# FaspDevTeam/faspsolver

Hardware: AMD Instinct MI355X
Metric: AMG-PCG solve DOF/s (3D 7-pt Poisson 256^3, classical AMG V(1,1) w-Jacobi + PCG, rtol 1e-8) (higher is better)
Workload: dtype f64

## Files before the change

### faspsolver_amd/__init__.py

```python
import ctypes as C
import os
import subprocess

import numpy as np

from . import _types as T
from ._types import *

_HERE = os.path.dirname(os.path.abspath(__file__))
LIB_PATH = os.environ.get("FASP_HIP_LIB") or os.path.join(_HERE, "libfasp_hip.so")
_lib = None

EXPORTS = [
    "fasp_param_amg_init", "fasp_param_solver_init", "fasp_solver_dcsr_krylov_amg",
    "fasp_blas_dcsr_mxv", "fasp_blas_dcsr_aAxpy", "fasp_blas_darray_dotprod",
    "fasp_blas_darray_norm2", "fasp_blas_darray_norminf", "fasp_blas_darray_axpy",
    "fasp_blas_darray_axpby", "fasp_smoother_dcsr_jacobi",
    "fasp_blas_dbsr_mxv", "fasp_blas_dbsr_aAxpy", "fasp_dbsr_getdiaginv", "fasp_smoother_dbsr_jacobi1",
    "fasp_solver_dbsr_pcg", "fasp_solver_dbsr_pbcgs", "fasp_solver_dbsr_pgmres", "fasp_solver_dbsr_pvgmres",
    "fasp_solver_dbsr_pvfgmres", "fasp_hip_bsr_precond_setup", "fasp_hip_bsr_precond_fct", "fasp_hip_bsr_precond_free",
    "fasp_hip_param_input", "fasp_fwrapper_dcsr_krylov_amg_", "fasp_dcsrvec_read2", "fasp_dvec_read",
    "fasp_dbsr_read", "fasp_dcoo_read", "fasp_dcoo_read1", "fasp_dcoo_shift_read", "fasp_dmtx_read", "fasp_dmtxsym_read", "fasp_dvec_write", "fasp_dcsr_write_coo", "fasp_dcsrvec_write2", "fasp_fwrapper_dcsr_amg_", "fasp_fwrapper_dbsr_krylov_amg_", "fasp_hip_free_bsr", "fasp_hip_comm_selftest", "fasp_hip_amg_kernel_info", "fasp_hip_coarse_kernel_info", "fasp_hip_bsr_coarse_kernel_info", "fasp_hip_coding_selftest", "fasp_solver_amg", "fasp_solver_famg", "fasp_hip_amg_solve", "fasp_precond_diag", "fasp_precond_dbsr_diag", "fasp_solver_dcsr_itsolver", "fasp_solver_dcsr_krylov", "fasp_solver_dcsr_krylov_diag", "fasp_solver_dbsr_itsolver", "fasp_solver_dbsr_krylov", "fasp_solver_dbsr_krylov_diag", "fasp_hip_mxv_csr", "fasp_hip_mxv_bsr", "fasp_solver_matfree_init", "fasp_solver_pcg", "fasp_solver_pbcgs", "fasp_solver_pgcg", "fasp_solver_pminres", "fasp_solver_pgmres", "fasp_solver_pvgmres", "fasp_solver_pvfgmres", "fasp_solver_itsolver", "fasp_solver_krylov", "fasp_solver_dcsr_pcg", "fasp_solver_dcsr_pminres", "fasp_solver_dcsr_pgcg", "fasp_solver_dcsr_pgcr", "fasp_solver_dcsr_pbcgs", "fasp_solver_dcsr_pgmres", "fasp_solver_dcsr_pvgmres",
    "fasp_solver_dcsr_pvfgmres", "fasp_hip_precond_setup", "fasp_hip_precond_fct", "fasp_hip_precond_free",
    "fasp_hip_time_bsr_mxv", "fasp_solver_dbsr_krylov_amg", "fasp_hip_bsr_amg_create", "fasp_hip_bsr_amg_create_host",
    "fasp_hip_bsr_amg_destroy", "fasp_hip_bsr_amg_num_levels", "fasp_hip_bsr_amg_get_matrix",
    "fasp_hip_bsr_amg_get_diaginv", "fasp_hip_bsr_solve",
    "fasp_hip_set_device", "fasp_hip_device_count", "fasp_hip_device_identity", "fasp_hip_available",
    "fasp_hip_amg_create", "fasp_hip_amg_create_host", "fasp_hip_amg_upload",
    "fasp_hip_amg_destroy", "fasp_hip_amg_num_levels", "fasp_hip_amg_get_matrix",
    "fasp_hip_amg_get_cfmark", "fasp_hip_solve", "fasp_hip_set_rhs", "fasp_hip_set_guess",
    "fasp_hip_solve_resident", "fasp_hip_get_solution", "fasp_hip_device_synchronize",
    "fasp_hip_precond_amg",
    "fasp_hip_poisson7pt", "fasp_hip_aniso27pt", "fasp_hip_free_system", "fasp_hip_time_kernel", "fasp_hip_measure_ceilings", "fasp_hip_amg_publish", "fasp_hip_amg_attach", "fasp_hip_amg_unpublish",
    "fasp_precond_setup", "fasp_precond_amg", "fasp_precond_famg", "fasp_precond_amli", "fasp_precond_namli", "fasp_amg_data_create", "fasp_amg_data_free", "fasp_param_amg_to_prec", "fasp_param_prec_to_amg", "fasp_mem_free", "fasp_mem_calloc", "fasp_dvec_alloc", "fasp_dvec_set", "fasp_dvec_free", "fasp_dvec_create", "fasp_dcsr_create", "fasp_dcsr_free", "fasp_smoother_dcsr_gs", "fasp_smoother_dcsr_sor", "fasp_smoother_dcsr_L1diag",
    "fasp_hip_tune", "fasp_hip_comm_unique_id", "fasp_hip_comm_init", "fasp_hip_comm_finalize",
    "fasp_hip_comm_rank", "fasp_hip_comm_size", "fasp_hip_version", "fasp_hip_comm_init_shm",
    "fasp_hip_dist_plan", "fasp_hip_dist_level_info", "fasp_hip_dist_get_matrix",
    "fasp_hip_dist_get_list",
    "fasp_blas_dcsr_vmv", "fasp_blas_dcsr_mxv_agg", "fasp_blas_dcsr_aAxpy_agg", "fasp_blas_darray_ax",
    "fasp_blas_darray_axpyz", "fasp_blas_darray_norm1", "fasp_darray_cp", "fasp_darray_set", "fasp_dvec_isnan",
    "fasp_hip_time_matrix", "fasp_hip_bsr_dist_info", "fasp_hip_seq_schedule_selftest", "fasp_hip_seq_chain_selftest", "fasp_hip_cluster_order", "fasp_hip_permute_csr", "fasp_hip_comm_init_ipc", "fasp_hip_comm_stats", "fasp_hip_comm_timing", "fasp_hip_estream_selftest", "fasp_hip_sell_selftest", "fasp_hip_csr_plan", "fasp_hip_level_op", "fasp_hip_matrix_op", "fasp_hip_matrix_traits",
    "fasp_param_ilu_init", "fasp_ilu_data_create", "fasp_ilu_data_free", "fasp_mem_iludata_check", "fasp_ilu_dcsr_setup",
    "fasp_precond_ilu", "fasp_precond_ilu_forward", "fasp_precond_ilu_backward", "fasp_solver_dcsr_krylov_ilu",
    "fasp_solver_dcsr_krylov_ilu_M", "fasp_smoother_dcsr_ilu", "fasp_fwrapper_dcsr_krylov_ilu_",
    "fasp_hip_ilu_resident_count", "fasp_hip_ilu_time",
    "fasp_ilu_dbsr_setup", "fasp_precond_dbsr_ilu", "fasp_solver_dbsr_krylov_ilu", "fasp_smoother_dbsr_ilu",
    "fasp_fwrapper_dbsr_krylov_ilu_",
    "fasp_hip_bsr_amg_get_ilu", "fasp_hip_bsr_amg_ilu_info", "fasp_hip_bsr_amg_ilu_smooth_time",
    "fasp_hip_bsr_sweep", "fasp_hip_csr_sweep",
    "fasp_blas_dcsr_rap", "fasp_hip_dcsr_rap", "fasp_hip_rap_info", "fasp_hip_rap_device_count", "fasp_hip_rap_time",
    "fasp_dstr_create", "fasp_dstr_alloc", "fasp_dstr_free", "fasp_dstr_cp", "fasp_format_dstr_dcsr", "fasp_dstr_read",
    "fasp_blas_dstr_aAxpy", "fasp_blas_dstr_mxv", "fasp_precond_dstr_diag", "fasp_solver_dstr_pcg", "fasp_solver_dstr_pbcgs",
    "fasp_solver_dstr_pminres", "fasp_solver_dstr_pgmres", "fasp_solver_dstr_pvgmres", "fasp_solver_dstr_itsolver",
    "fasp_solver_dstr_krylov", "fasp_solver_dstr_krylov_diag", "fasp_hip_mxv_str", "fasp_hip_str_form", "fasp_hip_time_str_mxv",
    "fasp_ilu_dstr_setup0", "fasp_ilu_dstr_setup1", "fasp_precond_dstr_ilu0", "fasp_precond_dstr_ilu1", "fasp_solver_dstr_krylov_ilu",
    "fasp_hip_str_ilu_form", "fasp_hip_str_ilu_apply", "fasp_hip_time_str_ilu",
    "fasp_smoother_dstr_jacobi", "fasp_smoother_dstr_jacobi1", "fasp_smoother_dstr_gs", "fasp_smoother_dstr_gs1",
    "fasp_smoother_dstr_gs_ascend", "fasp_smoother_dstr_gs_descend", "fasp_smoother_dstr_gs_order", "fasp_smoother_dstr_gs_cf",
    "fasp_smoother_dstr_sor", "fasp_smoother_dstr_sor1", "fasp_smoother_dstr_sor_ascend", "fasp_smoother_dstr_sor_descend",
    "fasp_smoother_dstr_sor_order", "fasp_smoother_dstr_sor_cf",
    "fasp_hip_str_sweep", "fasp_hip_str_sweep_form", "fasp_hip_str_sweep_levels", "fasp_hip_time_str_sweep",
    "fasp_generate_diaginv_block", "fasp_smoother_dstr_swz", "fasp_precond_dstr_blockgs", "fasp_solver_dstr_krylov_blockgs",
    "fasp_hip_str_swz", "fasp_hip_str_swz_levels", "fasp_hip_time_str_swz",
    "fasp_param_swz_init", "fasp_dcsr_sympart", "fasp_dcsr_shift", "fasp_sparse_mis", "fasp_swz_dcsr_setup", "fasp_dcsr_swz_forward",
    "fasp_dcsr_swz_backward", "fasp_precond_swz", "fasp_swz_data_free", "fasp_solver_dcsr_krylov_swz",
    "fasp_hip_csr_swz_levels", "fasp_hip_csr_swz", "fasp_hip_csr_swz_resident_count", "fasp_hip_time_csr_swz",
    "fasp_hip_csr_swz_runs", "fasp_hip_amg_get_swz", "fasp_hip_amg_swz_info", "fasp_hip_amg_swz_sweep_time", "fasp_hip_amg_swz_levels",
]


def build(verbose=False):
    cmd = ["make", "-C", os.path.join(_HERE, "csrc")]
    if not verbose:
        cmd.insert(1, "-s")
    subprocess.run(cmd, check=True)


def lib():
    global _lib
    if _lib is not None:
        return _lib
    if not os.path.exists(LIB_PATH):
        build()
    L = C.CDLL(LIB_PATH)
    P = C.POINTER
    L.fasp_param_amg_init.argtypes = [P(T.AMG_param)]
    L.fasp_param_solver_init.argtypes = [P(T.ITS_param)]
    L.fasp_solver_dcsr_krylov_amg.argtypes = [P(T.dCSRmat), P(T.dvector), P(T.dvector),
                                              P(T.ITS_param), P(T.AMG_param)]
    L.fasp_blas_dcsr_mxv.argtypes = [P(T.dCSRmat), T.c_double_p, T.c_double_p]
    L.fasp_blas_dcsr_aAxpy.argtypes = [C.c_double, P(T.dCSRmat), T.c_double_p, T.c_double_p]
    for f in ("fasp_blas_darray_dotprod", "fasp_blas_darray_norm2", "fasp_blas_darray_norminf"):
        getattr(L, f).restype = C.c_double
    L.fasp_blas_darray_dotprod.argtypes = [C.c_int, T.c_double_p, T.c_double_p]
    L.fasp_blas_darray_norm2.argtypes = [C.c_int, T.c_double_p]
    L.fasp_blas_darray_norminf.argtypes = [C.c_int, T.c_double_p]
    L.fasp_blas_darray_axpy.argtypes = [C.c_int, C.c_double, T.c_double_p, T.c_double_p]
    L.fasp_blas_darray_axpby.argtypes = [C.c_int, C.c_double, T.c_double_p, C.c_double,
                                         T.c_double_p]
    L.fasp_blas_dcsr_vmv.restype = C.c_double
    L.fasp_blas_dcsr_vmv.argtypes = [P(T.dCSRmat), T.c_double_p, T.c_double_p]
    L.fasp_blas_dcsr_mxv_agg.argtypes = [P(T.dCSRmat), T.c_double_p, T.c_double_p]
    L.fasp_blas_dcsr_aAxpy_agg.argtypes = [C.c_double, P(T.dCSRmat), T.c_double_p, T.c_double_p]
    L.fasp_blas_darray_ax.argtypes = [C.c_int, C.c_double, T.c_double_p]
    L.fasp_blas_darray_axpyz.argtypes = [C.c_int, C.c_double, T.c_double_p, T.c_double_p, T.c_double_p]
    L.fasp_blas_darray_norm1.restype = C.c_double
    L.fasp_blas_darray_norm1.argtypes = [C.c_int, T.c_double_p]
    L.fasp_darray_cp.argtypes = [C.c_int, T.c_double_p, T.c_double_p]
    L.fasp_darray_set.argtypes = [C.c_int, T.c_double_p, C.c_double]
    L.fasp_hip_time_matrix.restype = C.c_double
    L.fasp_hip_time_matrix.argtypes = [P(T.dCSRmat), C.c_int, C.c_int, P(C.c_int)]
    L.fasp_dvec_isnan.restype = C.c_short
    L.fasp_dvec_isnan.argtypes = [P(T.dvector)]
    L.fasp_smoother_dcsr_jacobi.argtypes = [P(T.dvector), C.c_int, C.c_int, C.c_int,
                                            P(T.dCSRmat), P(T.dvector), C.c_int, C.c_double]
    L.fasp_blas_dbsr_mxv.argtypes = [P(T.dBSRmat), T.c_double_p, T.c_double_p]
    L.fasp_blas_dbsr_aAxpy.argtypes = [C.c_double, P(T.dBSRmat), T.c_double_p, T.c_double_p]
    L.fasp_dbsr_getdiaginv.argtypes = [P(T.dBSRmat)]
    L.fasp_dbsr_getdiaginv.restype = T.dvector
    L.fasp_smoother_dbsr_jacobi1.argtypes = [P(T.dBSRmat), P(T.dvector), P(T.dvector), T.c_double_p]
    L.fasp_hip_bsr_sweep.argtypes = [P(T.dBSRmat), T.c_double_p, T.c_double_p, T.c_double_p, C.c_int, C.c_int, C.c_double,
                                     P(C.c_int)]
    L.fasp_hip_csr_sweep.argtypes = [P(T.dCSRmat), P(C.c_int), C.c_int, C.c_int, C.c_double, C.c_int, T.c_double_p, T.c_double_p,
                                     P(C.c_int)]
    L.fasp_hip_time_bsr_mxv.argtypes = [P(T.dBSRmat), C.c_int]
    L.fasp_hip_time_bsr_mxv.restype = C.c_double
    L.fasp_solver_dcsr_pcg.argtypes = [P(T.dCSRmat), P(T.dvector), P(T.dvector), P(T.precond), C.c_double,
                                       C.c_double, C.c_int, C.c_short, C.c_short]
    L.fasp_solver_dcsr_pbcgs.argtypes = L.fasp_solver_dcsr_pcg.argtypes
    L.fasp_solver_dcsr_pminres.argtypes = L.fasp_solver_dcsr_pcg.argtypes
    L.fasp_solver_dcsr_pgcg.argtypes = L.fasp_solver_dcsr_pcg.argtypes
    L.fasp_solver_dcsr_pvgmres.argtypes = [P(T.dCSRmat), P(T.dvector), P(T.dvector), P(T.precond), C.c_double,
                                           C.c_double, C.c_int, C.c_short, C.c_short, C.c_short]
    L.fasp_solver_dcsr_pvfgmres.argtypes = L.fasp_solver_dcsr_pvgmres.argtypes
    L.fasp_solver_dcsr_pgmres.argtypes = L.fasp_solver_dcsr_pvgmres.argtypes
    L.fasp_solver_dcsr_pgcr.argtypes = L.fasp_solver_dcsr_pvgmres.argtypes
    L.fasp_hip_precond_setup.argtypes = [P(T.dCSRmat), P(T.AMG_param)]
    L.fasp_hip_precond_setup.restype = P(T.precond)
    L.fasp_hip_precond_free.argtypes = [P(T.precond)]
    L.fasp_hip_precond_free.restype = None
    L.fasp_hip_precond_fct.argtypes = [T.c_double_p, T.c_double_p, C.c_void_p]
    L.fasp_hip_precond_fct.restype = None
    L.fasp_solver_dbsr_pcg.argtypes = [P(T.dBSRmat), P(T.dvector), P(T.dvector), P(T.precond), C.c_double,
                                       C.c_double, C.c_int, C.c_short, C.c_short]
    L.fasp_solver_dbsr_pbcgs.argtypes = L.fasp_solver_dbsr_pcg.argtypes
    L.fasp_solver_dbsr_pvgmres.argtypes = [P(T.dBSRmat), P(T.dvector), P(T.dvector), P(T.precond), C.c_double,
                                           C.c_double, C.c_int, C.c_short, C.c_short, C.c_short]
    L.fasp_solver_dbsr_pgmres.argtypes = L.fasp_solver_dbsr_pvgmres.argtypes
    L.fasp_solver_dbsr_pvfgmres.argtypes = L.fasp_solver_dbsr_pvgmres.argtypes
    L.fasp_hip_bsr_precond_setup.argtypes = [P(T.dBSRmat), P(T.AMG_param)]
    L.fasp_hip_bsr_precond_setup.restype = P(T.precond)
    L.fasp_hip_bsr_precond_free.argtypes = [P(T.precond)]
    L.fasp_hip_bsr_precond_free.restype = None
    L.fasp_hip_bsr_precond_fct.argtypes = [T.c_double_p, T.c_double_p, C.c_void_p]
    L.fasp_hip_bsr_precond_fct.restype = None
    L.fasp_dcsrvec_read2.argtypes = [C.c_char_p, C.c_char_p, P(T.dCSRmat), P(T.dvector)]
    L.fasp_dvec_read.argtypes = [C.c_char_p, P(T.dvector)]
    L.fasp_dbsr_read.argtypes = [C.c_char_p, P(T.dBSRmat)]
    L.fasp_hip_free_bsr.argtypes = [P(T.dBSRmat)]
    L.fasp_hip_free_bsr.restype = None
    L.fasp_hip_param_input.argtypes = [C.c_char_p, P(T.ITS_param), P(T.AMG_param)]
    L.fasp_fwrapper_dcsr_krylov_amg_.argtypes = [P(C.c_int), P(C.c_int), T.c_int_p, T.c_int_p, T.c_double_p,
                                                 T.c_double_p, T.c_double_p, P(C.c_double), P(C.c_int), P(C.c_int)]
    L.fasp_fwrapper_dcsr_krylov_amg_.restype = None
    L.fasp_hip_coding_selftest.argtypes = [P(T.dCSRmat), P(C.c_int)]
    L.fasp_hip_amg_kernel_info.argtypes = [C.c_void_p, C.c_int, C.c_int, P(C.c_int), P(C.c_double)]
    L.fasp_hip_coarse_kernel_info.argtypes = [C.c_void_p, P(C.c_int)]
    L.fasp_hip_bsr_coarse_kernel_info.argtypes = [C.c_void_p, P(C.c_int)]
    L.fasp_solver_amg.argtypes = [P(T.dCSRmat), P(T.dvector), P(T.dvector), P(T.AMG_param)]
    L.fasp_hip_amg_solve.argtypes = [C.c_void_p, P(T.dvector), P(T.dvector), P(T.AMG_param), T.c_double_p,
                                     C.c_int, P(T.fasp_hip_stats)]
    L.fasp_solver_dbsr_krylov_amg.argtypes = [P(T.dBSRmat), P(T.dvector), P(T.dvector), P(T.ITS_param),
                                              P(T.AMG_param)]
    L.fasp_hip_bsr_amg_create.argtypes = [P(C.c_void_p), P(T.dBSRmat), P(T.AMG_param)]
    L.fasp_hip_bsr_amg_create_host.argtypes = [P(C.c_void_p), P(T.dBSRmat), P(T.AMG_param)]
    L.fasp_hip_bsr_amg_destroy.argtypes = [C.c_void_p]
    L.fasp_hip_bsr_amg_destroy.restype = None
    L.fasp_hip_bsr_amg_num_levels.argtypes = [C.c_void_p]
    L.fasp_hip_bsr_amg_get_matrix.argtypes = [C.c_void_p, C.c_int, C.c_int, P(T.dBSRmat)]
    L.fasp_hip_bsr_amg_get_diaginv.argtypes = [C.c_void_p, C.c_int]
    L.fasp_hip_bsr_amg_get_diaginv.restype = T.c_double_p
    L.fasp_hip_bsr_solve.argtypes = [C.c_void_p, P(T.dvector), P(T.dvector), P(T.ITS_param), T.c_double_p,
                                     C.c_int, P(T.fasp_hip_stats)]
    L.fasp_hip_amg_create.argtypes = [P(C.c_void_p), P(T.dCSRmat), P(T.AMG_param)]
    L.fasp_hip_amg_create_host.argtypes = L.fasp_hip_amg_create.argtypes
    L.fasp_hip_amg_upload.argtypes = [C.c_void_p]
    L.fasp_hip_amg_destroy.argtypes = [C.c_void_p]
    L.fasp_hip_amg_destroy.restype = None
    L.fasp_hip_amg_num_levels.argtypes = [C.c_void_p]
    L.fasp_hip_amg_get_matrix.argtypes = [C.c_void_p, C.c_int, C.c_int, P(T.dCSRmat)]
    L.fasp_hip_amg_get_cfmark.argtypes = [C.c_void_p, C.c_int, P(T.ivector)]
    L.fasp_hip_solve.argtypes = [C.c_void_p, P(T.dvector), P(T.dvector), P(T.ITS_param),
                                 T.c_double_p, C.c_int, P(T.fasp_hip_stats)]
    L.fasp_hip_set_rhs.argtypes = [C.c_void_p, P(T.dvector)]
# ... 606 lines not shown
```

### faspsolver_amd/csrc/device_csr.hip.h

```cpp

struct DevCSR {
    int     row = 0, col = 0, nnz = 0;
    int*    ia  = nullptr;
    int*    ja  = nullptr;
    double* val = nullptr;
    int*    dpos = nullptr;
    bool    dup_diag = false;
    bool    sorted = false;
    int     lanes = 8;
    int     kind = 0;
    int     tile_rows = 256;
    int     wrows = 64, wcap = 512;
    unsigned char* code = nullptr;
    int*    rowbase = nullptr;
    int*    doff = nullptr;
    double* dval = nullptr;
    unsigned short* pat = nullptr;
    int*    pstart = nullptr;
    int*    plen = nullptr;
    int*    poff = nullptr;
    double* pval = nullptr;
    int     npat = 0, npent = 0;
    unsigned short* ja16 = nullptr;
    int*            jbase = nullptr;
    int     nxrows = -1;
    int     plane = 0;
    int     win_lo = 0, win_hi = -1;
    unsigned short* lja16 = nullptr;
    int*    tptr = nullptr;
    int*    tcols = nullptr;
    long long ntcols = 0;
    const int* bridge = nullptr;
    double*    bscratch = nullptr;
    int        bridge_dir = 0;
    int*       es_tab = nullptr;
    unsigned short* es_ja16 = nullptr;
    double*    es_part = nullptr;
    int        es_W = 0, es_nc = 0;
    unsigned*      sell_code = nullptr;
    int*           sell_meta = nullptr;
    unsigned char* sell_rlen = nullptr;
    double*        sell_tab = nullptr;
    int            sell_nv = 0, sell_obits = 0, sell_nslice = 0;
    long long      sell_slots = 0;
    void    release()
    {
        if (sell_code) (void)hipFree(sell_code);
        if (sell_meta) (void)hipFree(sell_meta);
        if (sell_rlen) (void)hipFree(sell_rlen);
        if (sell_tab) (void)hipFree(sell_tab);
        sell_code = nullptr; sell_meta = nullptr; sell_rlen = nullptr; sell_tab = nullptr; sell_nv = sell_obits = sell_nslice = 0; sell_slots = 0;
        if (es_tab) (void)hipFree(es_tab);
        if (es_part) (void)hipFree(es_part);
        if (es_ja16) (void)hipFree(es_ja16);
        es_tab = nullptr; es_part = nullptr; es_ja16 = nullptr; es_W = es_nc = 0;
        if (bscratch) (void)hipFree(bscratch);
        bscratch = nullptr; bridge = nullptr; bridge_dir = 0;
        if (lja16) (void)hipFree(lja16);
        if (tptr) (void)hipFree(tptr);
        if (tcols) (void)hipFree(tcols);
        lja16 = nullptr; tptr = nullptr; tcols = nullptr;
        nxrows = -1;
        if (ja16) (void)hipFree(ja16);
        ja16 = nullptr;
        if (jbase) (void)hipFree(jbase);
        jbase = nullptr;
        if (ia) (void)hipFree(ia);
        if (ja) (void)hipFree(ja);
        if (val) (void)hipFree(val);
        if (dpos) (void)hipFree(dpos);
        if (code) (void)hipFree(code);
        if (rowbase) (void)hipFree(rowbase);
        if (doff) (void)hipFree(doff);
        if (dval) (void)hipFree(dval);
        if (pat) (void)hipFree(pat);
        if (pstart) (void)hipFree(pstart);
        if (plen) (void)hipFree(plen);
        if (poff) (void)hipFree(poff);
        if (pval) (void)hipFree(pval);
        pat = nullptr; pstart = plen = poff = nullptr; pval = nullptr;
        ia = ja = dpos = rowbase = doff = nullptr; val = dval = nullptr; code = nullptr;
    }
};

static void pick_kernel(DevCSR& M)
{
    const double avg = M.row > 0 ? (double)M.nnz / M.row : 1.0;
    static const double stream_max = std::getenv("FASP_HIP_STREAM_MAX") ? std::atof(std::getenv("FASP_HIP_STREAM_MAX")) : 48.0;
    M.kind = avg <= stream_max ? 2 : 0;
    M.lanes = avg < 300.0 ? 16 : avg < 1000.0 ? 32 : 64;
    while (M.lanes < 64 && (double)M.row * M.lanes < 0.75 * MAXGRID * BLOCK) M.lanes *= 2;
    if (avg < 48.0) M.lanes = avg < 3.0 ? 2 : avg < 6.0 ? 4 : avg < 24.0 ? 8 : 16;
    static const int small_rows = std::getenv("FASP_HIP_SMALL_XFER_ROWS") ? std::atoi(std::getenv("FASP_HIP_SMALL_XFER_ROWS")) : 256 * 1024;
    if (M.kind == 2 && M.row != M.col && M.row < small_rows) M.kind = 0;
    int R = 256;
    while (R < STREAM_MAXR && R * 2 * avg <= 3072.0) R <<= 1;
    M.tile_rows = R;
    M.wrows = 64;
    M.wcap  = 512;
}

static bool g_oneshot_upload = false;
static bool compress_enabled()
{
    if (g_oneshot_upload) return false;
    static int en = -1;
    if (en < 0) { const char* e = std::getenv("FASP_HIP_COMPRESS"); en = (e && std::atoi(e) == 0) ? 0 : 1; }
    return en != 0;
}
struct PairKey { int off; unsigned long long bits; };
static inline unsigned pair_hash(int off, unsigned long long bits)
{
    unsigned long long h = bits * 0x9E3779B97F4A7C15ull + (unsigned long long)(unsigned)off * 0xC2B2AE3D27D4EB4Full;
    return (unsigned)(h >> 40);
}
static bool build_dict8(const HostCSR& M, std::vector<int>& doff, std::vector<double>& dval,
                        Buf<unsigned char>& code, Buf<int>& rowbase)
{
    const bool square = M.row == M.col;
    const int n = M.row;
    if (n <= 0 || M.nnz <= 0) return false;
    constexpr int SLOTS = 1024;
    struct Table {
        int      cnt = 0;
        int      slot_id[SLOTS];
        PairKey  keys[257];
        Table() { for (int& s : slot_id) s = -1; }
        int find_or_add(int off, unsigned long long bits, bool add)
        {
            unsigned h = pair_hash(off, bits) & (SLOTS - 1);
            for (;;) {
                const int id = slot_id[h];
                if (id < 0) {
                    if (!add || cnt >= 257) return -1;
                    keys[cnt] = PairKey{off, bits};
                    slot_id[h] = cnt;
                    return cnt++;
                }
                if (keys[id].off == off && keys[id].bits == bits) return id;
                h = (h + 1) & (SLOTS - 1);
            }
        }
    };
    auto base_of = [&](int r) { return square ? r : (M.ia[r] < M.ia[r + 1] ? M.ja[M.ia[r]] : 0); };
    auto bits_of = [](double v) { unsigned long long b; std::memcpy(&b, &v, 8); return b; };
    const int nt = omp_get_max_threads();
    std::vector<Table> local((size_t)nt);
    bool fail = false;
#pragma omp parallel num_threads(nt)
    {
        Table& T = local[(size_t)omp_get_thread_num()];
#pragma omp for schedule(static)
        for (int r = 0; r < n; ++r) {
            if (fail || T.cnt > 256) continue;
            const int base = base_of(r);
            for (int k = M.ia[r]; k < M.ia[r + 1]; ++k)
                if (T.find_or_add(M.ja[k] - base, bits_of(M.val[k]), true) < 0 || T.cnt > 256) { fail = true; break; }
        }
    }
    if (fail) return false;
    std::vector<PairKey> all;
    for (const Table& T : local) all.insert(all.end(), T.keys, T.keys + T.cnt);
    std::sort(all.begin(), all.end(), [](const PairKey& x, const PairKey& y) {
        return x.off != y.off ? x.off < y.off : x.bits < y.bits; });
    all.erase(std::unique(all.begin(), all.end(), [](const PairKey& x, const PairKey& y) {
        return x.off == y.off && x.bits == y.bits; }), all.end());
    if (all.size() > 256) return false;
    doff.assign(256, 0); dval.assign(256, 0.0);
    Table G;
    for (size_t i = 0; i < all.size(); ++i) {
        G.find_or_add(all[i].off, all[i].bits, true);
        doff[i] = all[i].off;
        std::memcpy(&dval[i], &all[i].bits, 8);
    }
    code.alloc((size_t)M.nnz);
    if (!square) rowbase.alloc((size_t)n);
#pragma omp parallel
    {
        Table T = G;
#pragma omp for schedule(static)
        for (int r = 0; r < n; ++r) {
            const int base = base_of(r);
            if (!square) rowbase[r] = base;
            for (int k = M.ia[r]; k < M.ia[r + 1]; ++k)
                code[k] = (unsigned char)T.find_or_add(M.ja[k] - base, bits_of(M.val[k]), false);
        }
    }
    return true;
}

static bool build_rowpat(const HostCSR& M, Buf<unsigned short>& pat, std::vector<int>& pstart, std::vector<int>& plen,
                         std::vector<int>& poff, std::vector<double>& pval, Buf<int>& rowbase)
{
    const bool square = M.row == M.col || M.row_aligned;
    const int n = M.row;
    if (n <= 0 || M.nnz <= 0) return false;
    if ((long long)M.col >= (1ll << 28)) return false;
    constexpr int MAXPAT = 65535, MAXENT = 1 << 20;
    auto base_of = [&](int r) { return square ? r : (M.ia[r] < M.ia[r + 1] ? M.ja[M.ia[r]] : 0); };
// ... 478 lines not shown
    const int ns = (n + 63) / 64;
    S.rlen.assign((size_t)n, 0);
    S.sptr.assign((size_t)ns + 1, 0);
    int toolong = 0;
#pragma omp parallel for schedule(static) reduction(+ : toolong)
    for (int s = 0; s < ns; ++s) {
        int W = 0;
        for (int r = s * 64; r < std::min(n, s * 64 + 64); ++r) {
            const int len = M.ia[r + 1] - M.ia[r];
            if (len > 255) { ++toolong; continue; }
            S.rlen[(size_t)r] = (unsigned char)len;
            W = std::max(W, len);
        }
        S.sptr[(size_t)s + 1] = W;
    }
    if (toolong) { why = 2; return false; }
    long long wsum = 0;
    for (int s = 0; s < ns; ++s) wsum += S.sptr[(size_t)s + 1];
    S.nslice = ns;
    S.slots = 64ll * wsum;
    if (S.slots * 100 > (long long)cap_percent * M.nnz || wsum >= (1ll << 30)) { why = 3; return false; }
    for (int s = 0; s < ns; ++s) S.sptr[(size_t)s + 1] += S.sptr[(size_t)s];
    constexpr int VSLOTS = 32768;
    struct VSet {
        std::vector<unsigned long long> key;
        std::vector<long long> cnt;
        std::vector<int> id;
        int n = 0;
        VSet() : key((size_t)VSLOTS, 0ull), cnt((size_t)VSLOTS, 0), id((size_t)VSLOTS, -1) {}
        static unsigned slot_of(unsigned long long b) { return (unsigned)((b * 0x9E3779B97F4A7C15ull) >> 49); }
        bool add(unsigned long long b, long long c)
        {
            unsigned s = slot_of(b);
            for (;;) {
                if (cnt[s] == 0) {
                    if (n >= SELL_MAXV) return false;
                    key[s] = b; cnt[s] = c; ++n;
                    return true;
                }
                if (key[s] == b) { cnt[s] += c; return true; }
                s = (s + 1) & (VSLOTS - 1);
            }
        }
        int slot(unsigned long long b) const
        {
            unsigned s = slot_of(b);
            for (;;) {
                if (cnt[s] == 0) return -1;
                if (key[s] == b) return (int)s;
                s = (s + 1) & (VSLOTS - 1);
            }
        }
    };
    auto bits_of = [](double v) { unsigned long long b; std::memcpy(&b, &v, 8); return b; };
    const int nt = std::max(1, std::min(omp_get_max_threads(), n / 4096 + 1));
    std::vector<VSet*> local((size_t)nt, nullptr);
    bool fail = false;
#pragma omp parallel num_threads(nt)
    {
        VSet* T = new VSet();
        local[(size_t)omp_get_thread_num()] = T;
#pragma omp for schedule(static)
        for (int r = 0; r < n; ++r) {
            if (fail) continue;
            for (int k = M.ia[r]; k < M.ia[r + 1]; ++k)
                if (!T->add(bits_of(M.val[k]), 1)) { fail = true; break; }
        }
    }
    VSet Gs;
    for (VSet* T : local) {
        if (T && !fail)
            for (int s = 0; s < VSLOTS && !fail; ++s)
                if (T->cnt[(size_t)s] && !Gs.add(T->key[(size_t)s], T->cnt[(size_t)s])) fail = true;
        delete T;
    }
    if (fail) { why = 4; return false; }
    std::vector<std::pair<long long, unsigned long long>> order;
    for (int s = 0; s < VSLOTS; ++s)
        if (Gs.cnt[(size_t)s]) order.emplace_back(-Gs.cnt[(size_t)s], Gs.key[(size_t)s]);
    std::sort(order.begin(), order.end());
    S.nv = (int)order.size();
    S.tab.resize(order.size());
    for (size_t i = 0; i < order.size(); ++i) std::memcpy(&S.tab[i], &order[i].second, 8);
    for (size_t i = 0; i < order.size(); ++i) Gs.id[(size_t)Gs.slot(order[i].second)] = (int)i;
    S.vbits = 0;
    while ((1ll << S.vbits) < S.nv) ++S.vbits;
    S.sbase.assign((size_t)ns, 0);
    int maxoff = 0;
#pragma omp parallel for schedule(static) reduction(max : maxoff)
    for (int s = 0; s < ns; ++s) {
        const int k0 = M.ia[s * 64], k1 = M.ia[std::min(n, s * 64 + 64)];
        if (k1 <= k0) continue;
        int lo = M.ja[k0], hi = lo;
        for (int k = k0 + 1; k < k1; ++k) { lo = std::min(lo, M.ja[k]); hi = std::max(hi, M.ja[k]); }
        S.sbase[(size_t)s] = lo;
        maxoff = std::max(maxoff, hi - lo);
    }
    S.obits = 1;
    while ((1ll << S.obits) <= maxoff) ++S.obits;
    if (S.vbits + S.obits > 32) { why = 5; return false; }
    S.code.alloc((size_t)std::max<long long>(S.slots, 1));
    bool lost = false;
#pragma omp parallel for schedule(static)
    for (int s = 0; s < ns; ++s) {
        const int W = S.sptr[(size_t)s + 1] - S.sptr[(size_t)s], base = S.sbase[(size_t)s];
        unsigned* cs = S.code.data() + (size_t)S.sptr[(size_t)s] * 64;
        for (int l = 0; l < 64; ++l) {
            const int r = s * 64 + l;
            const int kb = r < n ? M.ia[r] : 0, len = r < n ? M.ia[r + 1] - kb : 0;
            for (int k = 0; k < len; ++k) {
                const int sl = Gs.slot(bits_of(M.val[kb + k]));
                if (sl < 0) { lost = true; continue; }
                const int id = Gs.id[(size_t)sl];
                cs[(size_t)k * 64 + l] = ((unsigned)id << S.obits) | (unsigned)(M.ja[kb + k] - base);
            }
            for (int k = len; k < W; ++k) cs[(size_t)k * 64 + l] = 0u;
        }
    }
    if (lost) { why = 4; return false; }
    why = 0;
    return true;
}

static void sell_mxv_host(const SellHost& S, int nrow, const double* x, double* y)
{
    const unsigned omask = (1u << S.obits) - 1u;
    for (int s = 0; s < S.nslice; ++s) {
        const int W = S.sptr[(size_t)s + 1] - S.sptr[(size_t)s], base = S.sbase[(size_t)s];
        const unsigned* cs = S.code.data() + (size_t)S.sptr[(size_t)s] * 64;
        double acc[64];
        for (int l = 0; l < 64; ++l) acc[l] = 0.0;
        for (int k = 0; k < W; ++k)
            for (int l = 0; l < 64; ++l) {
                const int r = s * 64 + l;
                if (r >= nrow || k >= (int)S.rlen[(size_t)r]) continue;
                const unsigned c = cs[(size_t)k * 64 + l];
                acc[l] = acc[l] + S.tab[c >> S.obits] * x[base + (int)(c & omask)];
            }
        for (int l = 0; l < 64 && s * 64 + l < nrow; ++l) y[s * 64 + l] = acc[l];
    }
}
static void sell_decode_host(const SellHost& S, int nrow, int* ia, int* ja, double* val)
{
    const unsigned omask = (1u << S.obits) - 1u;
    ia[0] = 0;
    for (int r = 0; r < nrow; ++r) ia[r + 1] = ia[r] + (int)S.rlen[(size_t)r];
    for (int r = 0; r < nrow; ++r) {
        const int s = r >> 6, l = r & 63, base = S.sbase[(size_t)s];
        const unsigned* cs = S.code.data() + (size_t)S.sptr[(size_t)s] * 64;
        for (int k = 0; k < (int)S.rlen[(size_t)r]; ++k) {
            const unsigned c = cs[(size_t)k * 64 + l];
            ja[ia[r] + k] = base + (int)(c & omask);
            val[ia[r] + k] = S.tab[c >> S.obits];
        }
    }
}

static int upload_sell(const HostCSR& H, DevCSR& D)
{
    static const bool on = !(std::getenv("FASP_HIP_SELL") && std::atoi(std::getenv("FASP_HIP_SELL")) == 0);
    if (!on) return FASP_SUCCESS;
    static const bool timing = std::getenv("FASP_HIP_SETUP_TIMING") != nullptr;
    const double t0 = wall_seconds();
    SellHost S;
    int why = 0;
    const bool ok = build_sell(H, S, SELL_CAP_PERCENT, &why);
    if (timing) std::printf("        [sell %d x %d, %d nnz] %s (%d) %d values, %d + %d bits, %.3f slots per entry, %.3f s\n", H.row, H.col, H.nnz,
                            ok ? "coded" : "not coded", why, S.nv, S.vbits, S.obits, (double)S.slots / std::max(H.nnz, 1), wall_seconds() - t0);
    if (!ok) return FASP_SUCCESS;
    const size_t ns = (size_t)S.nslice;
    std::vector<int> meta(2 * ns + 1);
    std::copy(S.sptr.begin(), S.sptr.end(), meta.begin());
    std::copy(S.sbase.begin(), S.sbase.end(), meta.begin() + (long)ns + 1);
    HIPCK(hipMalloc(&D.sell_code, sizeof(unsigned) * (size_t)std::max<long long>(S.slots, 1)));
    HIPCK(hipMalloc(&D.sell_meta, sizeof(int) * meta.size()));
    HIPCK(hipMalloc(&D.sell_rlen, (size_t)H.row));
    HIPCK(hipMalloc(&D.sell_tab, sizeof(double) * (size_t)S.nv));
    HIPCK(hipMemcpy(D.sell_code, S.code.data(), sizeof(unsigned) * (size_t)S.slots, hipMemcpyHostToDevice));
    HIPCK(hipMemcpy(D.sell_meta, meta.data(), sizeof(int) * meta.size(), hipMemcpyHostToDevice));
    HIPCK(hipMemcpy(D.sell_rlen, S.rlen.data(), (size_t)H.row, hipMemcpyHostToDevice));
    HIPCK(hipMemcpy(D.sell_tab, S.tab.data(), sizeof(double) * (size_t)S.nv, hipMemcpyHostToDevice));
    D.sell_nv = S.nv; D.sell_obits = S.obits; D.sell_nslice = S.nslice; D.sell_slots = S.slots;
    return FASP_SUCCESS;
}

static int upload_csr(const HostCSR& H, DevCSR& D)
{
    D.row = H.row; D.col = H.col; D.nnz = H.nnz;
    HIPCK(hipMalloc(&D.ia, sizeof(int) * ((size_t)H.row + 1)));
    HIPCK(hipMalloc(&D.ja, sizeof(int) * std::max<size_t>(H.nnz, 1)));
    HIPCK(hipMalloc(&D.val, sizeof(double) * (std::max<size_t>(H.nnz, 1) + 2)));
    HIPCK(hipMemsetAsync(D.val + std::max<size_t>(H.nnz, 1), 0, sizeof(double) * 2, g_ctx.stream));
    HIPCK(hipMemcpyAsync(D.ia, H.ia.data(), sizeof(int) * ((size_t)H.row + 1), hipMemcpyHostToDevice, g_ctx.stream));
    pick_kernel(D);
    auto upload_plain = [&]() -> int {
        HIPCK(hipMemcpyAsync(D.ja, H.ja.data(), sizeof(int) * (size_t)H.nnz, hipMemcpyHostToDevice, g_ctx.stream));
        HIPCK(hipMemcpyAsync(D.val, H.val.data(), sizeof(double) * (size_t)H.nnz, hipMemcpyHostToDevice, g_ctx.stream));
        return 0;
    };
    if (compress_enabled() && H.nnz >= 4096 && (double)H.nnz <= 48.0 * H.row) {
        Buf<unsigned short> pat; Buf<int> prb;
        std::vector<int> pstart, plen, poff; std::vector<double> pval;
        static const bool rowpat_on = !(std::getenv("FASP_HIP_ROWPAT") && std::atoi(std::getenv("FASP_HIP_ROWPAT")) == 0);
        if (rowpat_on && build_rowpat(H, pat, pstart, plen, poff, pval, prb)) {
            D.npat = (int)pstart.size(); D.npent = (int)poff.size();
            HIPCK(hipMalloc(&D.pat, sizeof(unsigned short) * ((size_t)H.row + 2)));
            HIPCK(hipMalloc(&D.pstart, sizeof(int) * pstart.size()));
            HIPCK(hipMalloc(&D.plen, sizeof(int) * plen.size()));
            HIPCK(hipMemcpy(D.plen, plen.data(), sizeof(int) * plen.size(), hipMemcpyHostToDevice));
            HIPCK(hipMalloc(&D.poff, sizeof(int) * std::max<size_t>(poff.size(), 1)));
            HIPCK(hipMalloc(&D.pval, sizeof(double) * std::max<size_t>(pval.size(), 1)));
            HIPCK(hipMemset(D.pat + H.row, 0xff, sizeof(unsigned short) * 2));
            HIPCK(hipMemcpy(D.pat, pat.data(), sizeof(unsigned short) * (size_t)H.row, hipMemcpyHostToDevice));
            HIPCK(hipMemcpy(D.pstart, pstart.data(), sizeof(int) * pstart.size(), hipMemcpyHostToDevice));
            HIPCK(hipMemcpy(D.poff, poff.data(), sizeof(int) * poff.size(), hipMemcpyHostToDevice));
            HIPCK(hipMemcpy(D.pval, pval.data(), sizeof(double) * pval.size(), hipMemcpyHostToDevice));
            if (prb.n) {
                HIPCK(hipMalloc(&D.rowbase, sizeof(int) * ((size_t)H.row + 2)));
                HIPCK(hipMemcpy(D.rowbase, prb.data(), sizeof(int) * (size_t)H.row, hipMemcpyHostToDevice));
                const int nr = H.row, npair = (nr + 1) / 2;
                long long nx = 0;
#pragma omp parallel for schedule(static) reduction(+ : nx)
                for (int w0 = 0; w0 < nr; w0 += 128) {
                    const int    pm = std::min((w0 + 64) / 2, npair - 1);
                    const unsigned domA = pat[(size_t)2 * pm], domB = (2 * pm + 1 < nr) ? pat[(size_t)2 * pm + 1] : 0xffffu;
                    for (int r = w0; r < std::min(w0 + 128, nr); r += 2) {
                        const bool vb = r + 1 < nr;
                        if (!(vb && pat[r] == domA && pat[r + 1] == domB)) nx += vb ? 2 : 1;
                    }
                }
                if (nx * 4 <= nr) D.nxrows = (int)nx;
            } else {
                D.plane = grid_plane_of(poff, H.row);
                if (std::getenv("FASP_HIP_SETUP_TIMING")) std::printf("        [upload_csr %d x %d, %d nnz] %d row patterns; grid plane for the XCD strips: %d rows\n", H.row, H.col, H.nnz, (int)pstart.size(), D.plane);
                const int nr = H.row, npair = (nr + 1) / 2;
                long long nx = 0;
#pragma omp parallel for schedule(static) reduction(+ : nx)
                for (int w0 = 0; w0 < nr; w0 += 128) {
                    const unsigned dom = pat[(size_t)2 * std::min((w0 + 64) / 2, npair - 1)];
                    for (int r = w0; r < std::min(w0 + 128, nr); r += 2) {
                        const bool vb = r + 1 < nr;
                        if (!(vb && pat[r] == dom && pat[r + 1] == dom)) nx += vb ? 2 : 1;
                    }
                }
                if (nx * 4 <= nr) D.nxrows = (int)nx;
            }
            D.kind = 2;
            return upload_plain() < 0 ? ERROR_ALLOC_MEM : FASP_SUCCESS;
        }
        std::vector<int> doff; std::vector<double> dval;
        Buf<unsigned char> code; Buf<int> rowbase;
        if (build_dict8(H, doff, dval, code, rowbase)) {
            HIPCK(hipMalloc(&D.code, (size_t)H.nnz + 256));
            HIPCK(hipMalloc(&D.doff, sizeof(int) * 256));
            HIPCK(hipMalloc(&D.dval, sizeof(double) * 256));
            HIPCK(hipMemcpy(D.code, code.data(), (size_t)H.nnz, hipMemcpyHostToDevice));
            HIPCK(hipMemcpy(D.doff, doff.data(), sizeof(int) * 256, hipMemcpyHostToDevice));
            HIPCK(hipMemcpy(D.dval, dval.data(), sizeof(double) * 256, hipMemcpyHostToDevice));
            if (rowbase.n) {
                HIPCK(hipMalloc(&D.rowbase, sizeof(int) * (size_t)H.row));
                HIPCK(hipMemcpy(D.rowbase, rowbase.data(), sizeof(int) * (size_t)H.row, hipMemcpyHostToDevice));
            }
            D.kind = 2;
            return upload_plain() < 0 ? ERROR_ALLOC_MEM : FASP_SUCCESS;
        }
    }
    static const bool sort_long = !(std::getenv("FASP_HIP_SORT_LONG_ROWS") && std::atoi(std::getenv("FASP_HIP_SORT_LONG_ROWS")) == 0);
    static const int  sort_stream = std::getenv("FASP_HIP_SORT_STREAM") ? std::atoi(std::getenv("FASP_HIP_SORT_STREAM")) : 0;
    const double avg_len = H.row > 0 ? (double)H.nnz / H.row : 0.0;
    const bool do_sort = sort_long && !g_oneshot_upload && H.nnz > 0 && (D.kind == 0 || (D.kind == 2 && sort_stream > 0 && avg_len >= sort_stream));
    static const bool timing = std::getenv("FASP_HIP_SETUP_TIMING") != nullptr;
    double tp = wall_seconds();
    auto lap = [&](const char* what) {
        if (!timing) return;
        const double now = wall_seconds();
        std::printf("        [upload_csr %d x %d, %d nnz] %-10s %8.3f s\n", H.row, H.col, H.nnz, what, now - tp);
        tp = now;
    };
    if (do_sort && D.kind == 0) {
        int maxlen = 0;
#pragma omp parallel for schedule(static) reduction(max : maxlen)
        for (int i = 0; i < H.row; ++i) maxlen = std::max(maxlen, H.ia[i + 1] - H.ia[i]);
        if (g_device_sort && maxlen <= SORT_MAXLEN) {
            const int st = upload_sorted_on_device(H, D, maxlen);
            lap("device sort");
            return st < 0 ? st : build_estream(H.ia.data(), H.row, H.nnz, D);
        }
    }
    if (do_sort) {
        Buf<int> sj((size_t)H.nnz);
        Buf<double> sv((size_t)H.nnz);
        std::vector<int> dp;
        const bool square = H.row == H.col;
        if (square) dp.assign((size_t)H.row, -1);
#pragma omp parallel
        {
            std::vector<std::pair<int, double>> tmp;
#pragma omp for schedule(dynamic, 64)
            for (int i = 0; i < H.row; ++i) {
                const int kb = H.ia[i], ke = H.ia[i + 1];
                tmp.resize((size_t)(ke - kb));
                for (int k = kb; k < ke; ++k) tmp[(size_t)(k - kb)] = {H.ja[k], H.val[k]};
                std::stable_sort(tmp.begin(), tmp.end(),
                                 [](const std::pair<int, double>& x, const std::pair<int, double>& y) { return x.first < y.first; });
                for (int k = kb; k < ke; ++k) {
                    sj[k] = tmp[(size_t)(k - kb)].first; sv[k] = tmp[(size_t)(k - kb)].second;
                    if (square && sj[k] == i) dp[(size_t)i] = k;
                }
            }
        }
        lap("row sort");
        HIPCK(hipMemcpy(D.ja, sj.data(), sizeof(int) * (size_t)H.nnz, hipMemcpyHostToDevice));
        HIPCK(hipMemcpy(D.val, sv.data(), sizeof(double) * (size_t)H.nnz, hipMemcpyHostToDevice));
        lap("memcpy");
        if (square && D.kind == 2) {
            HIPCK(hipMalloc(&D.dpos, sizeof(int) * (size_t)std::max(H.row, 1)));
            HIPCK(hipMemcpy(D.dpos, dp.data(), sizeof(int) * (size_t)H.row, hipMemcpyHostToDevice));
        }
        D.sorted = true;
        if (upload_ja16(D, H.ia.data(), sj.data()) < 0) return ERROR_ALLOC_MEM;
        return build_estream(H.ia.data(), H.row, H.nnz, D);
    }
    if (upload_plain() < 0) return ERROR_ALLOC_MEM;
    if (D.kind == 2 && !g_oneshot_upload && build_xtile(H, D) < 0) return ERROR_ALLOC_MEM;
    if (D.kind == 2 && compress_enabled() && upload_sell(H, D) < 0) return ERROR_ALLOC_MEM;
    if (upload_ja16(D, H.ia.data(), H.ja.data()) < 0) return ERROR_ALLOC_MEM;
    return build_estream(H.ia.data(), H.row, H.nnz, D);
}

struct Tuning { int swz_run = -1, swz_run_width = 16, ilu_smooth_fused = 1, gen2 = 2, ws2_bpc = 3, maxgrid = -1, xcd = 16, nt = 1, kind = -1, lanes = -1, wrows = -1, wcap = -1, compress = 1, rpl = -1, lds_tab = 1, xcd_pat = 64, spcg_batch = 16, small_lds = 1, ja16 = 1, spcg_fused = 1, spcg_grid = 0, spcg_persist = 1, split_rows = 0, gs_multicolor = 0, seq_flow = 1, seq_strip_kb = 0, seq_jobs = 1, seq_spine = 1, seq_grid = 0, seq_chain = 1, seq_chain_n1 = 0, seq_chain_grid = 0, seq_chain_ref = 0, seq_test_hang = 0, seq_rest_lanes = 0, local_square = 1, fuse_zr = 1, fuse_presmooth = 1, seq_lanes = 0, xtile = 1, rp5_max = 45, rp_bpc = 5, rp_xcd = -1, rp_strip = 2, spcg_test_hang = 0, small_onewave = 4, lazy_coarse = 1, rp_stream = -1, renumber = 1, renumber_chunk = 262144, pcg_dev_beta = 1, spcg_spec = 1, ev_every = 4, pcg_fold = 1, seq_chain_touch = 8, seq_chain_touch_t1 = 1, seq_zero_skip = 1, estream = 1, es_dbg = 0, ilu_form = -1, str_ilu_form = -1, str_ilu_wgs = 0, str_sweep_form = -1, str_sweep_wgs = 0, sell = 1; };
static Tuning g_tune;

template <class K>
static int resident_blocks_per_cu(K kernel)
{
    static std::vector<std::pair<const void*, int>> cache;
    const void* key = reinterpret_cast<const void*>(kernel);
    for (const auto& e : cache)
        if (e.first == key) return e.second;
    int nb = 0;
    if (hipOccupancyMaxActiveBlocksPerMultiprocessor(&nb, kernel, BLOCK, 0) != hipSuccess || nb < 1) nb = 4;
    nb = std::min(nb, 8);
    cache.emplace_back(key, nb);
    return nb;
}

template <class K>
static int launch_persistent(K kernel, int ntiles, CsrArgs& a, int blocks_per_cu = 0)
{
    int cap = (blocks_per_cu > 0 ? std::min(blocks_per_cu, resident_blocks_per_cu(kernel)) : resident_blocks_per_cu(kernel)) * g_ctx.num_cu;
    if (g_tune.maxgrid > 0) cap = g_tune.maxgrid;
    cap = std::min(cap, MAXGRID);
    int grid = std::min(cap, ntiles);
    grid = std::max(8, (grid + 7) / 8 * 8);
    hipLaunchKernelGGL(kernel, dim3(grid), dim3(BLOCK), 0, g_ctx.stream, a);
    return grid;
}

enum CsrKernel : int {
    CK_ROWS_2 = 0, CK_ROWS_4, CK_ROWS_8, CK_ROWS_16, CK_ROWS_32, CK_ROWS_64,
    CK_WSTREAM_64_512, CK_WSTREAM_64_1024, CK_WSTREAM_32_512, CK_WSTREAM_32_1024,
    CK_ROWPAT_0_1, CK_ROWPAT_0_2, CK_ROWPAT_1_1, CK_ROWPAT_1_2, CK_ROWPAT_2_1, CK_ROWPAT_2_2,
    CK_DICT8_8, CK_DICT8_16, CK_DICT8_24,
    CK_ESTREAM_4, CK_ESTREAM_8, CK_ESTREAM_16, CK_ESTREAM_32,
    CK_ROWPAT4, CK_ROWPAT5, CK_LSTREAM, CK_XTILE, CK_SELL, CK_WSTREAM2
};
struct CsrPlan {
    CsrKernel kernel;
    int    family;
    int    tile_rows;
    int    bpc;
    int    xcd_map;
    int    tpp;
    int    nt;
    bool   ja16, jbase;
    bool   fused_zr;
    double bytes;
};
static CsrPlan plan_csr(const DevCSR& M, int op, bool windowed, bool want_partials, int rows = -1)
{
    CsrPlan p{};
    int kind = M.kind;
    if (rows < 0) rows = M.row;
    if (M.code && g_tune.compress) kind = 4;
    if (M.pat && g_tune.compress) kind = 5;
    if (g_tune.kind >= 0 && !(g_tune.kind == 4 && !M.code) && !(g_tune.kind == 5 && !M.pat)) kind = g_tune.kind;
    const int lanes = g_tune.lanes > 0 ? g_tune.lanes : M.lanes, wrows = g_tune.wrows > 0 ? g_tune.wrows : M.wrows, wcap = g_tune.wcap > 0 ? g_tune.wcap : M.wcap;
    const bool jac = op == OP_JACOBI, w64 = wrows == 64 && wcap == 512;
    const bool lstream_ok = g_tune.gen2 && kind == 2 && w64 && (double)M.nnz <= 7.6 * M.row;
    if (jac && kind != 0 && kind < 4 && (M.dup_diag || !M.dpos) && !lstream_ok) kind = 0;
    p.xcd_map = g_tune.xcd;
    p.nt = g_tune.nt | ((g_tune.rp_stream > 0 || (g_tune.rp_stream < 0 && (size_t)M.row * 8 > (size_t)96 << 20)) ? 4 : 0);
    p.ja16 = g_tune.ja16 && M.ja16; p.jbase = g_tune.ja16 && M.jbase;
    if (M.jbase && kind != 0) p.ja16 = p.jbase = false;
    if (kind == 1 || kind == 3) kind = 0;
    p.tile_rows = kind >= 4 ? BLOCK : kind == 2 ? 4 * wrows : BLOCK / lanes;
    auto ntiles = [&] { return (rows + p.tile_rows - 1) / p.tile_rows; };
    auto strips = [&] {
        const int rpb = p.tile_rows;
        if (!g_tune.rp_strip || M.plane < 8 * rpb || M.plane % (8 * rpb) != 0 || ntiles() < 4 * (M.plane / rpb)) return;
        p.xcd_map = -2; p.tpp = M.plane / rpb;
    };
    const double avg = M.row > 0 ? (double)M.nnz / M.row : 1.0, ptr_bytes = 4.0 * (M.row + 1.0), base_bytes = M.rowbase ? 4.0 * M.row : 0.0;
    const bool pair = kind == 5 && M.nxrows >= 0 && g_tune.rpl <= 0;
    p.bytes = kind == 5 ? 2.0 * M.row + base_bytes + 12.0 * M.npent : kind == 4 ? 1.0 * M.nnz + ptr_bytes + base_bytes : 12.0 * M.nnz + ptr_bytes;
    if (pair && g_tune.gen2 && !M.rowbase) {
        p.kernel = CK_ROWPAT4; p.family = 6; p.tile_rows = 2 * BLOCK;
        p.xcd_map = ntiles() >= 8 * 64 ? g_tune.rp_xcd : 16;
        if (p.xcd_map == -1) strips();
        p.bpc = p.xcd_map == -2 && g_tune.rp_bpc == 5 ? 3 : g_tune.rp_bpc;
        p.fused_zr = jac && want_partials;
    }
    else if (pair && g_tune.gen2 >= 2 && M.rowbase && !jac && op != OP_L1DIAG && (double)M.nnz <= 0.1 * g_tune.rp5_max * M.row) {
        p.kernel = CK_ROWPAT5; p.family = 9; p.tile_rows = 2 * BLOCK; p.bpc = 5;
        p.xcd_map = ntiles() >= 8 * 64 ? -1 : 16;
        if (g_tune.rp_strip >= 2) strips();
    }
    else if (kind == 5) {
        const int rpl = g_tune.rpl > 0 ? g_tune.rpl : 1;
        const bool lds = M.npat <= 512 && M.npent <= 2048 && g_tune.lds_tab != 0;
        const int T = !lds ? 0 : M.npat <= 64 && M.npent <= 512 && g_tune.lds_tab != 3 ? 2 : 1;
        p.kernel = CsrKernel(CK_ROWPAT_0_1 + 2 * T + (rpl != 1)); p.family = 5; p.tile_rows = BLOCK * rpl;
        if (g_tune.xcd_pat != 0) p.xcd_map = g_tune.xcd_pat;
        if (g_tune.xcd_pat == 64 && g_tune.rp_strip >= 2) strips();
    }
    else if (kind == 4) { p.kernel = avg <= 8.5 ? CK_DICT8_8 : avg <= 20.0 ? CK_DICT8_16 : CK_DICT8_24; p.family = 4; }
    else if (lstream_ok) { p.kernel = CK_LSTREAM; p.family = 7; p.bpc = 4; p.fused_zr = jac && want_partials; }
    else if (kind == 2 && g_tune.gen2 >= 2 && w64) {
        if (g_tune.xtile && M.lja16) {
            p.kernel = CK_XTILE; p.family = 10; p.bpc = 3;
            p.bytes = 10.0 * M.nnz + ptr_bytes + 4.0 * M.ntcols + 4.0 * ((M.row + 63) / 64 + 1.0);
        }
        else if (M.sell_code && g_tune.compress && g_tune.sell) {
            p.kernel = CK_SELL; p.family = 11; p.tile_rows = SELL_BLOCK;
            p.bytes = 4.0 * (double)M.sell_slots + 1.0 * M.row + 4.0 * (2.0 * M.sell_nslice + 1.0) + 8.0 * M.sell_nv;
        }
        else { p.kernel = CK_WSTREAM2; p.family = 8; p.bpc = g_tune.ws2_bpc; }
        p.fused_zr = jac && want_partials;
    }
    else if (kind == 2) {
        p.kernel = w64 ? CK_WSTREAM_64_512 : wrows == 64 ? CK_WSTREAM_64_1024 : wrows == 32 && wcap == 512 ? CK_WSTREAM_32_512 : CK_WSTREAM_32_1024; p.family = 2;
    }
    else {
        if (p.ja16) p.bytes = 10.0 * M.nnz + ptr_bytes + (p.jbase ? 4.0 * M.row : 0.0);
        const bool es_rule = g_tune.estream >= 2 || (g_tune.estream == 1 && (double)M.nnz < 256.0 * M.row);
        if (M.es_tab && es_rule && p.ja16 && !windowed && op != OP_MXV_DOT && !(jac && (want_partials || M.dup_diag)))
            p.kernel = avg >= 512.0 ? CK_ESTREAM_32 : avg >= 256.0 ? CK_ESTREAM_16 : avg >= 128.0 ? CK_ESTREAM_8 : CK_ESTREAM_4;
        else
            p.kernel = lanes == 2 ? CK_ROWS_2 : lanes == 4 ? CK_ROWS_4 : lanes == 8 ? CK_ROWS_8 : lanes == 16 ? CK_ROWS_16 : lanes == 32 ? CK_ROWS_32 : CK_ROWS_64;
    }
    return p;
}
static int kernel_family(const DevCSR& M, double* matrix_bytes)
{
    const CsrPlan p = plan_csr(M, OP_MXV, false, false);
    if (matrix_bytes) *matrix_bytes = p.bytes;
    return p.family;
}

template <int OP>
static int launch_sell(const DevCSR& M, CsrArgs& a)
{
    a.sell_code = M.sell_code; a.sell_sptr = M.sell_meta; a.sell_sbase = M.sell_meta + M.sell_nslice + 1; a.sell_rlen = M.sell_rlen;
    a.sell_tab = M.sell_tab; a.sell_nv = M.sell_nv; a.sell_obits = M.sell_obits;
    const size_t lds = sizeof(double) * ((size_t)M.sell_nv + SELL_NW);
    static bool attr_set = false;
    if (!attr_set) {
        (void)hipFuncSetAttribute(reinterpret_cast<const void*>(k_csr_sell<OP>), hipFuncAttributeMaxDynamicSharedMemorySize, (int)(sizeof(double) * (SELL_MAXV + SELL_NW)));
        attr_set = true;
    }
    static std::vector<std::pair<size_t, int>> cache;
    int nb = 0;
    for (const auto& e : cache)
        if (e.first == lds) nb = e.second;
    if (nb == 0) {
        if (hipOccupancyMaxActiveBlocksPerMultiprocessor(&nb, k_csr_sell<OP>, SELL_BLOCK, lds) != hipSuccess || nb < 1) nb = 1;
        nb = std::min(nb, 2);
        cache.emplace_back(lds, nb);
    }
    int cap = nb * g_ctx.num_cu;
    if (g_tune.maxgrid > 0) cap = g_tune.maxgrid;
    cap = std::min(cap, MAXGRID);
    int grid = std::min(cap, a.ntiles);
    grid = std::max(8, (grid + 7) / 8 * 8);
    hipLaunchKernelGGL(k_csr_sell<OP>, dim3(grid), dim3(SELL_BLOCK), lds, g_ctx.stream, a);
    return grid;
}

template <int OP>
static int launch_rowpat5(CsrArgs& a)
{
    if constexpr (OP == OP_JACOBI || OP == OP_L1DIAG) { (void)a; return 0; }
    else return launch_persistent(k_csr_rowpat5<OP>, a.ntiles, a, 5);
}

constexpr int WIN_ALIGN = DIST_WIN_ALIGN;
struct RowWin { int lo = 0, hi = -1, goff = 0; };

__global__ __launch_bounds__(BLOCK) void k_bridge_gather(int n, const int* __restrict__ perm, const double* __restrict__ s, double* __restrict__ y,
                                                         double* __restrict__ zx, const double* __restrict__ zdiag, double zomega)
{
    for (int k = blockIdx.x * BLOCK + threadIdx.x; k < n; k += gridDim.x * BLOCK) {
        const double v = s[perm[k]];
        y[k] = v;
        if (zx) { const double di = zdiag[k]; zx[k] = (fabs(di) > 1e-20) ? (1 - zomega) * 0.0 + zomega * v / di : 0.0; }
    }
}
__global__ __launch_bounds__(BLOCK) void k_bridge_scatter(int n, const int* __restrict__ perm, const double* __restrict__ x, double* __restrict__ s)
{
    for (int k = blockIdx.x * BLOCK + threadIdx.x; k < n; k += gridDim.x * BLOCK) s[perm[k]] = x[k];
}

template <int OP>
static int launch_csr(const DevCSR& M0, CsrArgs a, RowWin win = RowWin())
{
    if (M0.bridge && win.hi < 0) {
        DevCSR Mn = M0;
        Mn.bridge = nullptr; Mn.bscratch = nullptr; Mn.bridge_dir = 0;
        if (M0.bridge_dir == 1 && OP == OP_MXV) {
            CsrArgs b = a;
            b.y = M0.bscratch; b.zx = nullptr; b.zdiag = nullptr;
            const int G = launch_csr<OP>(Mn, b);
            const int grid = std::max(1, std::min(MAXGRID, (M0.row + BLOCK - 1) / BLOCK));
            hipLaunchKernelGGL(k_bridge_gather, dim3(grid), dim3(BLOCK), 0, g_ctx.stream, M0.row, M0.bridge, (const double*)M0.bscratch, a.y, a.zx, a.zdiag, a.zomega);
            return G;
        }
        if (M0.bridge_dir == 2 && (OP == OP_ADD || OP == OP_SUB || OP == OP_AXPY || OP == OP_MXV)) {
            const int grid = std::max(1, std::min(MAXGRID, (M0.col + BLOCK - 1) / BLOCK));
            hipLaunchKernelGGL(k_bridge_scatter, dim3(grid), dim3(BLOCK), 0, g_ctx.stream, M0.col, M0.bridge, a.x, M0.bscratch);
            CsrArgs b = a;
            b.x = M0.bscratch;
            return launch_csr<OP>(Mn, b);
        }
        std::fprintf(stderr, "### ERROR: fasp_hip: operation %d on a transfer operator with a numbering bridge (direction %d)\n", (int)OP, M0.bridge_dir);
        std::abort();
    }
    if (win.hi < 0 && g_tune.split_rows > 0 && M0.row >= 4 * WIN_ALIGN) {
        const int lo = std::min(g_tune.split_rows, M0.row / 4) / WIN_ALIGN * WIN_ALIGN, hi = (M0.row - lo) / WIN_ALIGN * WIN_ALIGN;
        RowWin w; w.lo = lo; w.hi = hi; w.goff = 0;
        int G = launch_csr<OP>(M0, a, w);
        w.lo = 0; w.hi = lo; w.goff = G;
        G += launch_csr<OP>(M0, a, w);
        w.lo = hi; w.hi = M0.row; w.goff = G;
        return G + launch_csr<OP>(M0, a, w);
    }
    const DevCSR& M = M0;
    const int w_lo = win.hi >= 0 ? win.lo : 0, w_hi = win.hi >= 0 ? std::min(win.hi, M0.row) : M0.row;
    if (w_hi <= w_lo && win.hi >= 0) return 0;
    if (a.partials) a.partials += win.goff;
    const CsrPlan p = plan_csr(M, OP, win.hi >= 0 || g_tune.split_rows > 0, a.partials != nullptr, w_hi - w_lo);
    const int rpb = p.tile_rows;
    if (win.hi >= 0 && rpb > 0 && (w_lo % rpb) != 0) {
        std::fprintf(stderr, "### ERROR: fasp_hip: row window at %d with a kernel tile of %d rows (a tuning knob broke the window alignment)\n", w_lo, rpb);
        std::abort();
    }
    a.nrow = w_hi; a.row_lo = w_lo; a.tile0 = w_lo / rpb;
    a.ntiles = (w_hi - w_lo + rpb - 1) / rpb; a.tiles_per_xcd = (a.ntiles + 7) / 8;
    a.xcd_map = p.xcd_map; a.nt = p.nt;
    if (p.tpp) { a.tpp = p.tpp; a.tiles_per_xcd = p.tpp / 8; }
    a.ia = M.ia; a.ja = M.ja; a.val = M.val; a.dpos = M.dpos;
    a.ja16 = p.ja16 ? M.ja16 : nullptr; a.jbase = p.jbase ? M.jbase : nullptr;
    if (p.family == 5 || p.family == 6 || p.family == 9) {
        a.pat = M.pat; a.pstart = M.pstart; a.plen = M.plen; a.poff = M.poff; a.pval = M.pval; a.rowbase = M.rowbase;
        a.npat = M.npat; a.npent = M.npent; a.ncol = M.col;
    }
    if (p.family == 4) { a.code = M.code; a.rowbase = M.rowbase; a.doff = M.doff; a.dval = M.dval; }
    if (p.kernel == CK_XTILE) { a.lja16 = M.lja16; a.tptr = M.tptr; a.tcols = M.tcols; }
#define PERSIST(...) return launch_persistent(__VA_ARGS__, a.ntiles, a, p.bpc)
    switch (p.kernel) {
        case CK_ROWS_2:  PERSIST(k_csr_rows<2, OP>);
        case CK_ROWS_4:  PERSIST(k_csr_rows<4, OP>);
        case CK_ROWS_8:  PERSIST(k_csr_rows<8, OP>);
        case CK_ROWS_16: PERSIST(k_csr_rows<16, OP>);
        case CK_ROWS_32: PERSIST(k_csr_rows<32, OP>);
        case CK_ROWS_64: PERSIST(k_csr_rows<64, OP>);
        case CK_WSTREAM_64_512:  PERSIST(k_csr_wstream<OP, 64, 512>);
        case CK_WSTREAM_64_1024: PERSIST(k_csr_wstream<OP, 64, 1024>);
        case CK_WSTREAM_32_512:  PERSIST(k_csr_wstream<OP, 32, 512>);
        case CK_WSTREAM_32_1024: PERSIST(k_csr_wstream<OP, 32, 1024>);
        case CK_ROWPAT_0_1: PERSIST(k_csr_rowpat<OP, 0, 1>);
        case CK_ROWPAT_0_2: PERSIST(k_csr_rowpat<OP, 0, 2>);
        case CK_ROWPAT_1_1: PERSIST(k_csr_rowpat<OP, 1, 1>);
        case CK_ROWPAT_1_2: PERSIST(k_csr_rowpat<OP, 1, 2>);
        case CK_ROWPAT_2_1: PERSIST(k_csr_rowpat<OP, 2, 1>);
        case CK_ROWPAT_2_2: PERSIST(k_csr_rowpat<OP, 2, 2>);
        case CK_DICT8_8:  PERSIST(k_csr_dict8<OP, 8>);
        case CK_DICT8_16: PERSIST(k_csr_dict8<OP, 16>);
        case CK_DICT8_24: PERSIST(k_csr_dict8<OP, 24>);
        case CK_ROWPAT4:  PERSIST(k_csr_rowpat4<OP>);
        case CK_ROWPAT5:  return launch_rowpat5<OP>(a);
        case CK_LSTREAM:  PERSIST(k_csr_lstream<OP, 512>);
        case CK_XTILE:    PERSIST(k_csr_xtile<OP>);
        case CK_SELL:     return launch_sell<OP>(M, a);
        case CK_WSTREAM2: PERSIST(k_csr_wstream2<OP>);
        default: break;
    }
#undef PERSIST
    const int W = M.es_W, nc = M.es_nc, lanes = 4 << (p.kernel - CK_ESTREAM_4);
    a.es_wc = M.es_tab; a.es_centry = a.es_wc + W + 1; a.es_crow = a.es_centry + nc + 1; a.es_hw0 = a.es_crow + nc + 1; a.es_np = a.es_hw0 + W;
    a.es_part = M.es_part; a.es_cnt = reinterpret_cast<unsigned*>(M.es_part + 2 * (size_t)W);
    a.es_cbase = M.es_ja16 ? a.es_np + W : nullptr; a.es_ja16 = M.es_ja16;
    static bool attr_set = false;
#define ES_ATTR(LL) (void)hipFuncSetAttribute(reinterpret_cast<const void*>(k_csr_estream<LL, OP>), hipFuncAttributeMaxDynamicSharedMemorySize, ES_LDS_BYTES)
    if (!attr_set) { ES_ATTR(32); ES_ATTR(16); ES_ATTR(8); ES_ATTR(4); attr_set = true; }
#undef ES_ATTR
#define ES_LAUNCH(LL) hipLaunchKernelGGL((k_csr_estream<LL, OP>), dim3(W / 4), dim3(BLOCK), ES_LDS_BYTES, g_ctx.stream, a)
#ifdef FASP_LAB_DEBUG
    if (OP == OP_MXV && g_tune.es_dbg) {
#define ES_DBG(LL, DD) do { (void)hipFuncSetAttribute(reinterpret_cast<const void*>(k_csr_estream<LL, OP_MXV, DD>), hipFuncAttributeMaxDynamicSharedMemorySize, ES_LDS_BYTES); hipLaunchKernelGGL((k_csr_estream<LL, OP_MXV, DD>), dim3(W / 4), dim3(BLOCK), ES_LDS_BYTES, g_ctx.stream, a); } while (0)
        const int dd = g_tune.es_dbg;
        if (lanes == 32) { if (dd == 1) ES_DBG(32, 1); else if (dd == 2) ES_DBG(32, 2); else if (dd == 3) ES_DBG(32, 3); else if (dd == 4) ES_DBG(32, 4); else ES_DBG(32, 7); }
        else if (lanes == 16) { if (dd == 1) ES_DBG(16, 1); else if (dd == 2) ES_DBG(16, 2); else if (dd == 3) ES_DBG(16, 3); else if (dd == 4) ES_DBG(16, 4); else ES_DBG(16, 7); }
        else if (lanes == 8) { if (dd == 1) ES_DBG(8, 1); else if (dd == 2) ES_DBG(8, 2); else if (dd == 3) ES_DBG(8, 3); else if (dd == 4) ES_DBG(8, 4); else ES_DBG(8, 7); }
        else { if (dd == 1) ES_DBG(4, 1); else if (dd == 2) ES_DBG(4, 2); else if (dd == 3) ES_DBG(4, 3); else if (dd == 4) ES_DBG(4, 4); else ES_DBG(4, 7); }
#undef ES_DBG
        return W / 4;
    }
#endif
    static const bool es_log = std::getenv("FASP_HIP_ES_LOG") != nullptr;
    if (es_log) { std::fprintf(stderr, "[es rank %d] op %d rows %d cols %d nnz %d W %d chunks %d lanes %d rel %d x %p y %p b %p\n", comm_rank(), (int)OP, M.row, M.col, M.nnz, W, nc, lanes, M.es_ja16 != nullptr, (const void*)a.x, (void*)a.y, (const void*)a.b); std::fflush(stderr); }
    if (lanes == 32) ES_LAUNCH(32); else if (lanes == 16) ES_LAUNCH(16); else if (lanes == 8) ES_LAUNCH(8); else ES_LAUNCH(4);
#undef ES_LAUNCH
    if (es_log) { const hipError_t e = hipStreamSynchronize(g_ctx.stream); std::fprintf(stderr, "[es rank %d] done: %s\n", comm_rank(), hipGetErrorString(e)); std::fflush(stderr); }
    return W / 4;
}

static void d_mxv(const DevCSR& A, const double* x, double* y)
{
    CsrArgs a{}; a.x = x; a.y = y;
    launch_csr<OP_MXV>(A, a);
}
static void d_resid(const DevCSR& A, const double* x, const double* b, double* y)
{
    CsrArgs a{}; a.x = x; a.y = y; a.b = b;
    launch_csr<OP_RESID>(A, a);
}
static void d_aAxpy(double alpha, const DevCSR& A, const double* x, double* y)
{
    CsrArgs a{}; a.x = x; a.y = y; a.alpha = alpha;
    if (alpha == 1.0) launch_csr<OP_ADD>(A, a);
    else if (alpha == -1.0) launch_csr<OP_SUB>(A, a);
    else launch_csr<OP_AXPY>(A, a);
}

static void d_finalize_to(int G, int nq, unsigned maxmask, double* out, bool dist)
{
    hipLaunchKernelGGL(k_finalize, dim3(1), dim3(BLOCK), 0, g_ctx.stream, g_ctx.d_partials, G, nq,
                       maxmask, out);
    if (dist && comm_size() > 1 && comm_allreduce(out, nq, maxmask, g_ctx.stream) < 0) comm_mark_failed();
}
static void d_finalize(int G, int nq, unsigned maxmask, int slot, bool dist)
{
    d_finalize_to(G, nq, maxmask, g_ctx.d_red + slot, dist);
}
static int fetch_red(int slot, int nq, double* out)
{
    HIPCK(hipMemcpyAsync(g_ctx.h_red + slot, g_ctx.d_red + slot, sizeof(double) * nq,
                         hipMemcpyDeviceToHost, g_ctx.stream));
    HIPCK(hipStreamSynchronize(g_ctx.stream));
    for (int q = 0; q < nq; ++q) out[q] = g_ctx.h_red[slot + q];
    if (comm_failed()) {
        std::fprintf(stderr, "### ERROR: fasp_hip: rank %d: a collective failed; the iteration is abandoned\n", comm_rank());
        return ERROR_MISC;
    }
    return FASP_SUCCESS;
}
static int d_dot_to(int n, const double* x, const double* y, int slot, bool dist)
{
    const int G = vec_grid(n);
    hipLaunchKernelGGL(k_dot, dim3(G), dim3(BLOCK), 0, g_ctx.stream, n, x, y, g_ctx.d_partials);
    d_finalize(G, 1, 0u, slot, dist);
    return 0;
}
static int d_dot(int n, const double* x, const double* y, double* out, bool dist = false)
{
    const int G = vec_grid(n);
    hipLaunchKernelGGL(k_dot, dim3(G), dim3(BLOCK), 0, g_ctx.stream, n, x, y, g_ctx.d_partials);
    d_finalize(G, 1, 0u, 0, dist);
    return fetch_red(0, 1, out);
}
static int d_norms(int n, const double* x, double* out, bool dist = false)
{
    const int G = vec_grid(n);
    hipLaunchKernelGGL(k_norms, dim3(G), dim3(BLOCK), 0, g_ctx.stream, n, x, g_ctx.d_partials);
    d_finalize(G, 2, 0x2u, 0, dist);
    return fetch_red(0, 2, out);
}
static void d_axpy(int n, double a, const double* x, double* y)
{
    hipLaunchKernelGGL(k_axpy, dim3(vec_grid(n / 2 + 1)), dim3(BLOCK), 0, g_ctx.stream, n, a, x, y);
}
static void d_axpby(int n, double a, const double* x, double b, double* y)
{
    hipLaunchKernelGGL(k_axpby, dim3(vec_grid(n / 2 + 1)), dim3(BLOCK), 0, g_ctx.stream, n, a, x, b, y);
}
```

### faspsolver_amd/csrc/hierarchy.hip.h

```cpp

struct DevLevel {
    DevCSR  A, P, R;
    double* diag = nullptr;
    double* l1   = nullptr;
    double *b = nullptr, *xa = nullptr, *xb = nullptr, *w = nullptr;
    double* x  = nullptr;
    double* xo = nullptr;
    bool    x_zero = true;
    bool    presmoothed = false;
    double* halo_pending = nullptr;
    bool    owns_b = true;
    bool    replicated = true;
    int     nloc = 0;
    int     nvec = 0;
    int     row0 = 0;
    int     nglobal = 0;
    std::vector<int> send_off, recv_off;
    int*    d_send_idx = nullptr;
    double* d_sendbuf  = nullptr;
    bool    has_halo() const { return !replicated && nvec > nloc; }
    struct Sched {
        bool built = false, multicolor = false; int* d_order = nullptr; int* d_ptr = nullptr; std::vector<int> ptr;
        int ns = 0, L = 1, LR = 1, pfmax = 1, kt = 0, par = 1, nstrips = 0, nchunk = 0, maxent = 0; bool nolower = false, flow_ok = false, rowlevels = false, independent = false; int nrows = 0, nvirt = 0, nclasses = 0; long long nghost = 0, slot_bytes = 0;
        std::vector<int> cptr;
// ... 196 lines not shown

template <int OP>
static int dist_launch(DevLevel& V, const DevCSR& M, CsrArgs a, const DevLevel* Out = nullptr)
{
    double* v = const_cast<double*>(a.x);
    if (V.replicated && (!Out || Out->replicated) && comm_size() > 1) return rep_launch<OP>(M, a);
    if (V.replicated || comm_size() <= 1 || V.send_off.empty()) return launch_csr<OP>(M, a);
    if (!g_halo_overlap || M.win_hi < 0) {
        if (halo_exchange(V, v) < 0) return -1;
        return launch_csr<OP>(M, a);
    }
    bool local_ok = hipEventRecord(g_ctx.ev_ready, g_ctx.stream) == hipSuccess &&
                    hipStreamWaitEvent(g_ctx.comm_stream, g_ctx.ev_ready, 0) == hipSuccess;
    if (!local_ok) {
        comm_mark_failed();
        (void)hipStreamSynchronize(g_ctx.stream);
        (void)halo_exchange(V, v);
        (void)launch_csr<OP>(M, a);
        return -1;
    }
    RowWin w;
    w.lo = M.win_lo; w.hi = M.win_hi; w.goff = 0;
    int G = launch_csr<OP>(M, a, w);
    const int hst = halo_exchange(V, v, g_ctx.comm_stream);
    if (hipEventRecord(g_ctx.ev_halo, g_ctx.comm_stream) != hipSuccess ||
        hipStreamWaitEvent(g_ctx.stream, g_ctx.ev_halo, 0) != hipSuccess) {
        comm_mark_failed();
        (void)hipStreamSynchronize(g_ctx.comm_stream);
        local_ok = false;
    }
    w.lo = 0; w.hi = M.win_lo; w.goff = G;
    G += launch_csr<OP>(M, a, w);
    w.lo = M.win_hi; w.hi = M.row; w.goff = G;
    G += launch_csr<OP>(M, a, w);
    return (hst < 0 || !local_ok) ? -1 : G;
}

static bool renumber_param_ok(const AMG_param& p)
{
    return (p.smoother == SMOOTHER_JACOBI || p.smoother == SMOOTHER_L1DIAG) &&
           (p.cycle_type == V_CYCLE || p.cycle_type == W_CYCLE || p.cycle_type == VW_CYCLE || p.cycle_type == WV_CYCLE) &&
           p.coarse_scaling != 1 && p.AMG_type == CLASSIC_AMG;
}
static bool renumber_allowed(const fasp_hip_amg* h)
{
    if (g_oneshot_upload) return false;
    return g_tune.renumber != 0 && comm_size() == 1 && renumber_param_ok(h->param);
}
static int renumber_conflict(const fasp_hip_amg* h, const AMG_param& p)
{
    bool any = false;
    for (const auto& pm : h->perm) any = any || !pm.empty();
    if (!any || renumber_param_ok(p)) return FASP_SUCCESS;
    std::printf("### ERROR: fasp_hip: this hierarchy was uploaded for an order-independent smoother (its mid levels are renumbered); "
                "smoother %d / cycle %d / coarse_scaling %d need the natural order -- set them before the setup, or "
                "fasp_hip_tune(\"renumber\", 0)\n", (int)p.smoother, (int)p.cycle_type, (int)p.coarse_scaling);
    return ERROR_INPUT_PAR;
}
static bool dev_coded(const DevCSR& M) { return M.pat != nullptr || M.code != nullptr; }

static int upload_transfer(fasp_hip_amg* h, int l, const DistLevel* DLp)
{
    const HostLevel& HL = h->H.L[l];
    DevLevel& D = h->L[l];
    const bool rep = !DLp || DLp->replicated;
    const std::vector<int>* pf = (size_t)l < h->perm.size() && !h->perm[(size_t)l].empty() ? &h->perm[(size_t)l] : nullptr;
    const std::vector<int>* pc = (size_t)l + 1 < h->perm.size() && !h->perm[(size_t)l + 1].empty() ? &h->perm[(size_t)l + 1] : nullptr;
    const bool bridged = pc && !pf && dev_coded(D.A);
    if (bridged) {
        if (upload_csr(HL.P, D.P) < 0) return ERROR_ALLOC_MEM;
        if (upload_csr(HL.R, D.R) < 0) return ERROR_ALLOC_MEM;
        DevLevel& C = h->L[(size_t)l + 1];
        if (!C.d_perm) {
            HIPCK(hipMalloc(&C.d_perm, sizeof(int) * pc->size()));
            HIPCK(hipMemcpy(C.d_perm, pc->data(), sizeof(int) * pc->size(), hipMemcpyHostToDevice));
        }
        HIPCK(hipMalloc(&D.R.bscratch, sizeof(double) * pc->size()));
        HIPCK(hipMalloc(&D.P.bscratch, sizeof(double) * pc->size()));
        D.R.bridge = C.d_perm; D.R.bridge_dir = 1;
        D.P.bridge = C.d_perm; D.P.bridge_dir = 2;
    } else if (pf || pc) {
        std::vector<int> invf, invc;
        if (pf) { invf.resize(pf->size()); for (size_t k = 0; k < pf->size(); ++k) invf[(size_t)(*pf)[k]] = (int)k; }
        if (pc) { invc.resize(pc->size()); for (size_t k = 0; k < pc->size(); ++k) invc[(size_t)(*pc)[k]] = (int)k; }
        HostCSR T;
        permute_csr(HL.P, pf ? pf->data() : nullptr, pc ? invc.data() : nullptr, T);
        if (upload_csr(T, D.P) < 0) return ERROR_ALLOC_MEM;
        HIPCK(hipStreamSynchronize(g_ctx.stream));
        permute_csr(HL.R, pc ? pc->data() : nullptr, pf ? invf.data() : nullptr, T);
        if (upload_csr(T, D.R) < 0) return ERROR_ALLOC_MEM;
        HIPCK(hipStreamSynchronize(g_ctx.stream));
    } else {
        if (upload_csr(rep ? HL.P : DLp->P, D.P) < 0) return ERROR_ALLOC_MEM;
        if (upload_csr(rep ? HL.R : DLp->R, D.R) < 0) return ERROR_ALLOC_MEM;
    }
    if (D.A.plane > 0 && D.R.row > 0 && D.R.col > 0) {
        D.P.plane = D.A.plane;
        const long long pr = (long long)D.A.plane * D.R.row;
        if (pr % D.R.col == 0) D.R.plane = (int)(pr / D.R.col);
    }
    if (!rep) {
        D.R.win_lo = DLp->winR[0]; D.R.win_hi = DLp->winR[1];
        D.P.win_lo = DLp->winP[0]; D.P.win_hi = DLp->winP[1];
    }
    return FASP_SUCCESS;
}

static int upload_level(fasp_hip_amg* h, int l, const DistLevel* DLp)
{
    const HostLevel& HL = h->H.L[l];
    DevLevel& D = h->L[l];
    const bool rep = !DLp || DLp->replicated;
    D.replicated = rep;
    D.nloc = rep ? HL.A.row : DLp->nloc; D.row0 = rep ? 0 : DLp->row0; D.nglobal = HL.A.row;
    D.nvec = rep ? HL.A.row : DLp->nloc + (int)DLp->ghosts.size();
    const HostCSR& A = rep ? HL.A : DLp->A;
    static const bool timing = std::getenv("FASP_HIP_SETUP_TIMING") != nullptr;
    double tp = wall_seconds();
    auto lap = [&](const char* what) {
        if (!timing) return;
        const double now = wall_seconds();
        std::printf("    [upload level %d] %-10s %8.3f s\n", l, what, now - tp);
        tp = now;
    };
    const bool renum = renumber_allowed(h);
    if (h->perm.size() < h->L.size()) h->perm.resize(h->L.size());
    HostCSR Aperm;
    const HostCSR* Adev = &A;
    if (!rep && g_tune.local_square) {
        HostCSR view;
        view.row = A.row; view.col = A.col; view.nnz = A.nnz; view.row_aligned = true;
        view.ia.view(const_cast<int*>(A.ia.data()), A.ia.n); view.ja.view(const_cast<int*>(A.ja.data()), A.ja.n); view.val.view(const_cast<double*>(A.val.data()), A.val.n);
        if (upload_csr(view, D.A) < 0) return ERROR_ALLOC_MEM;
    } else {
        bool want = renum && rep && l > 0 && HL.has_coarse && !HL.SWZ && A.row >= 4096 && A.row <= 2000000 && (g_tune.renumber >= 2 || !dev_coded(h->L[(size_t)l - 1].A));
        bool uploaded = false;
        if (want && compress_enabled() && (double)A.nnz <= 48.0 * A.row) {
            if (upload_csr(A, D.A) < 0) return ERROR_ALLOC_MEM;
            if (dev_coded(D.A)) { want = false; uploaded = true; }
            else { HIPCK(hipStreamSynchronize(g_ctx.stream)); D.A.release(); D.A = DevCSR(); }
        }
        if (want) {
            std::vector<int>& pm = h->perm[(size_t)l];
            cluster_order(A, std::max(4096, g_tune.renumber_chunk), pm);
            std::vector<int> inv(pm.size());
            for (size_t k = 0; k < pm.size(); ++k) inv[(size_t)pm[k]] = (int)k;
            permute_csr(A, pm.data(), inv.data(), Aperm);
            Adev = &Aperm;
            lap("renumber");
        }
        if (!uploaded && upload_csr(*Adev, D.A) < 0) return ERROR_ALLOC_MEM;
    }
    lap("A");
    if (renum) {
        if (l > 0 && h->H.L[(size_t)l - 1].has_coarse && !h->L[(size_t)l - 1].P.ia) {
            const int st = upload_transfer(h, l - 1, nullptr);
            if (st < 0) return st;
            lap("P, R of the level above");
        }
    } else if (HL.has_coarse) {
        const int st = upload_transfer(h, l, DLp);
        if (st < 0) return st;
        lap("P, R");
    }
    if (!rep) { D.A.win_lo = DLp->winA[0]; D.A.win_hi = DLp->winA[1]; }
    HIPCK(hipStreamSynchronize(g_ctx.stream));
    lap("sync");
    if (upload_diag(*Adev, D) < 0) return ERROR_ALLOC_MEM;
    lap("diag");
    { const int st = swz_level_upload(h, l); if (st < 0) return st; }
    lap("Schwarz");
    const size_t n = D.nvec;
    if (l > 0) { if (alloc_vec(&D.b, n) < 0) return ERROR_ALLOC_MEM; }
    else D.owns_b = false;
    if (alloc_vec(&D.xa, n) < 0 || alloc_vec(&D.xb, n) < 0 || alloc_vec(&D.w, n) < 0) return ERROR_ALLOC_MEM;
    D.x = D.xa; D.xo = D.xb; D.x_zero = true;
    if (!rep) {
        D.send_off = DLp->send_off; D.recv_off = DLp->recv_off;
        const size_t ns = DLp->send_idx.size();
        HIPCK(hipMalloc(&D.d_send_idx, sizeof(int) * std::max<size_t>(ns, 1)));
        HIPCK(hipMalloc(&D.d_sendbuf, sizeof(double) * std::max<size_t>(ns, 1)));
        if (ns) HIPCK(hipMemcpy(D.d_send_idx, DLp->send_idx.data(), sizeof(int) * ns, hipMemcpyHostToDevice));
    }
    return FASP_SUCCESS;
}

static int upload_hierarchy(fasp_hip_amg* h)
{
    HostThreads team;
    const double t0 = wall_seconds();
    const int nl = (int)h->H.L.size();
    h->L.resize(nl);
    int min_rows = 200000;
    if (const char* e = std::getenv("FASP_HIP_DIST_MIN_ROWS")) min_rows = std::atoi(e);
    const bool seq_ok = g_seq_partition && h->param.smoother != SMOOTHER_CG && h->param.smoother != SMOOTHER_JACOBIF;
    if (h->param.smoother != SMOOTHER_JACOBI && h->param.smoother != SMOOTHER_L1DIAG && h->param.smoother != SMOOTHER_POLY && !seq_ok) min_rows = 2147483647;
    if (h->param.cycle_type == AMLI_CYCLE || h->param.cycle_type == NL_AMLI_CYCLE) min_rows = 2147483647;
    {
        h->level_cycle_type.assign((size_t)nl, h->param.cycle_type);
        h->level_cycle_type[0] = 0;
        if (h->param.AMG_type == UA_AMG) {
            const double cplxmax = 3.0, xsi = 0.6, eta = xsi / ((1 - xsi) * (cplxmax - 1));
            int icum = 1;
            h->level_cycle_type[0] = 1;
            h->level_cycle_type[(size_t)nl - 1] = 0;
            for (int lvl = 1; lvl < nl - 1; ++lvl) {
                const double fracratio = (double)h->H.L[lvl].A.nnz / h->H.L[0].A.nnz;
                int ct = (int)(std::pow(xsi, (double)lvl) / (eta * fracratio * icum));
                ct = std::max(1, std::min(2, ct));
                h->level_cycle_type[(size_t)lvl] = ct;
                icum = icum * ct;
            }
        }
    }
    {
        const int st = build_dist_plan(h->H, comm_rank(), comm_size(), min_rows, h->dist);
        if (st < 0) return st;
    }
    h->distributed = !h->dist.L[0].replicated;
    for (int l = 0; l < nl && comm_size() > 1; ++l)
        if (h->H.L[l].SWZ) {
            std::printf("### ERROR: fasp_hip: Schwarz smoothing (SWZ_levels > 0) has no multi-GPU path\n");
            return ERROR_INPUT_PAR;
        }
    for (int l = 0; l < nl; ++l) {
        if (h->L[l].A.ia) continue;
        const int st = upload_level(h, l, &h->dist.L[l]);
        if (st < 0) return st;
    }
    const size_t m = h->L[0].nvec;
    if (alloc_vec(&h->b, m) < 0 || alloc_vec(&h->u, m) < 0 || alloc_vec(&h->p, m) < 0 ||
        alloc_vec(&h->t, m) < 0 || alloc_vec(&h->r, m) < 0) return ERROR_ALLOC_MEM;
    HIPCK(hipMemsetAsync(h->u, 0, sizeof(double) * m, g_ctx.stream));
    HIPCK(hipMemsetAsync(h->p, 0, sizeof(double) * m, g_ctx.stream));
    const size_t mc = h->L[nl - 1].nvec;
    if (alloc_vec(&h->cp, mc) < 0 || alloc_vec(&h->cr, mc) < 0 || alloc_vec(&h->ct, mc) < 0 ||
        alloc_vec(&h->cbest, mc) < 0) return ERROR_ALLOC_MEM;
    h->ev.resize(64);
    for (auto& e : h->ev) { HIPCK(hipEventCreate(&e.a)); HIPCK(hipEventCreate(&e.b)); }
    HIPCK(hipStreamSynchronize(g_ctx.stream));
    for (auto& DL : h->dist.L) { if (!seq_ok) DL.A = HostCSR(); DL.P = HostCSR(); DL.R = HostCSR(); }
    h->upload_seconds = wall_seconds() - t0;
    return FASP_SUCCESS;
}
```

### faspsolver_amd/csrc/kernels.hip.h

```cpp
#pragma once

#include <hip/hip_runtime.h>

namespace fasp {

constexpr int BLOCK   = 256;
constexpr int MAXGRID = 2048;

enum RowOp : int {
    OP_MXV = 0,
    OP_RESID,
    OP_ADD,
    OP_SUB,
    OP_AXPY,
    OP_JACOBI,
    OP_L1DIAG,
    OP_MXV_DOT
};

struct CsrArgs {
    int           nrow;
    const int*    ia;
    const int*    ja;
    const double* val;
    const double* x;
    double*       y;
    const double* b;
    const double* diag;
    const int*    dpos;
    const double* dotv;
    double*       partials;
    double        alpha;
    double        omega;
    int           ntiles;
    int           tiles_per_xcd;
    int           tpp;
    int           xcd_map;
    int           nt;
    const unsigned char* code;
    const int*    rowbase;
    const int*    doff;
    const double* dval;
    const unsigned short* pat;
    const int*    pstart;
    const int*    plen;
    const int*    poff;
    const double* pval;
    int           npat, npent;
    int           ncol;
    const int*    stop;
    const int*    mark;
    const unsigned short* ja16;
    const int*            jbase;
    int           tile0, row_lo;
    double*       zx;
    const double* zdiag;
    double        zomega;
    const unsigned short* lja16;
    const int*    tptr;
    const int*    tcols;
    const int*    es_wc;
    const int*    es_centry;
    const int*    es_crow;
    const int*    es_hw0;
    const int*    es_np;
    const int*    es_cbase;
    const unsigned short* es_ja16;
    double*       es_part;
    unsigned*     es_cnt;
    const unsigned*      sell_code;
    const int*           sell_sptr;
    const int*           sell_sbase;
    const unsigned char* sell_rlen;
    const double*        sell_tab;
    int                  sell_nv, sell_obits;
};

__device__ __forceinline__ void zx_store(const CsrArgs& a, int r, double s)
{
    if (a.zx) {
        const double di = a.zdiag[r];
        a.zx[r] = (fabs(di) > 1e-20) ? (1 - a.zomega) * 0.0 + a.zomega * s / di : 0.0;
    }
}

__device__ __forceinline__ double l1_or_jacobi_f(const CsrArgs& a, int r, double t, double d, double xi)
{
    if (a.mark) return a.mark[r] == 0 ? xi + a.omega * t / d : xi;
    return (fabs(d) > 1e-20) ? xi + t / d : xi;
}

__device__ __forceinline__ int ld_ja(const CsrArgs& a, int k)
{
    if (a.ja16) return a.nt ? (int)__builtin_nontemporal_load(a.ja16 + k) : (int)a.ja16[k];
    return a.nt ? __builtin_nontemporal_load(a.ja + k) : a.ja[k];
}
__device__ __forceinline__ double ld_val(const CsrArgs& a, int k)
{
    return a.nt ? __builtin_nontemporal_load(a.val + k) : a.val[k];
}
__device__ __forceinline__ int tile_vmax(const CsrArgs& a)
{
    if (a.xcd_map == -2) return 8 * a.tiles_per_xcd * ((a.ntiles + a.tpp - 1) / a.tpp);
    if (a.xcd_map < 0) return 8 * a.tiles_per_xcd;
    if (a.xcd_map <= 0) return a.ntiles;
    const int span = 8 * a.xcd_map;
    return (a.ntiles + span - 1) / span * span;
}
__device__ __forceinline__ int tile_of(const CsrArgs& a, int v)
{
    if (a.xcd_map == -2) {
        const int q = v >> 3, z = q / a.tiles_per_xcd;
        return z * a.tpp + (v & 7) * a.tiles_per_xcd + (q - z * a.tiles_per_xcd);
    }
    if (a.xcd_map < 0) return (v & 7) * a.tiles_per_xcd + (v >> 3);
    if (a.xcd_map <= 0) return v;
    const int G = a.xcd_map;
    const int xcd = v & 7, q = v >> 3;
    int chunk, within;
    if ((G & (G - 1)) == 0) { const int sh = __ffs(G) - 1; chunk = q >> sh; within = q & (G - 1); }
    else { chunk = q / G; within = q - chunk * G; }
    return (chunk * 8 + xcd) * G + within;
}

template <int W>
__device__ __forceinline__ double subwave_sum(double v)
{
#pragma unroll
    for (int off = W / 2; off > 0; off >>= 1) v += __shfl_down(v, off, W);
    return v;
}

__device__ __forceinline__ void wave_lds_sync()
{
    __builtin_amdgcn_fence(__ATOMIC_RELEASE, "workgroup");
    __builtin_amdgcn_wave_barrier();
    __builtin_amdgcn_fence(__ATOMIC_ACQUIRE, "workgroup");
}

__device__ __forceinline__ double block_sum(double v, double* lds )
{
    v = subwave_sum<64>(v);
    const int wave = threadIdx.x >> 6, lane = threadIdx.x & 63;
    __syncthreads();
    if (lane == 0) lds[wave] = v;
    __syncthreads();
    double r = 0.0;
    if (threadIdx.x == 0) r = ((lds[0] + lds[1]) + lds[2]) + lds[3];
    return r;
}
__device__ __forceinline__ double block_max(double v, double* lds)
{
#pragma unroll
    for (int off = 32; off > 0; off >>= 1) v = fmax(v, __shfl_down(v, off, 64));
    const int wave = threadIdx.x >> 6, lane = threadIdx.x & 63;
    __syncthreads();
    if (lane == 0) lds[wave] = v;
    __syncthreads();
    double r = 0.0;
    if (threadIdx.x == 0) r = fmax(fmax(lds[0], lds[1]), fmax(lds[2], lds[3]));
    return r;
}

template <int L, int OP>
__global__ __launch_bounds__(BLOCK) void k_csr_rows(CsrArgs a)
{
    if (a.stop && *a.stop) return;
    constexpr int RPB = BLOCK / L;
    const int sl   = threadIdx.x & (L - 1);
    const int rloc = threadIdx.x / L;
    const int vmax = tile_vmax(a);
    double acc = 0.0;

    for (int v = blockIdx.x; v < vmax; v += gridDim.x) {
        const int t = tile_of(a, v);
        if (t >= a.ntiles) continue;
        const int r = (t + a.tile0) * RPB + rloc;
        if (r < a.nrow) {
            const int kb = a.ia[r], ke = a.ia[r + 1];
            const int jb = a.jbase ? a.jbase[r] : 0;
            double s = 0.0;
            int k = kb + sl;
            for (; k + 3 * L < ke; k += 4 * L) {
                const int    c0 = jb + ld_ja(a, k);
                const int    c1 = jb + ld_ja(a, k + L);
                const int    c2 = jb + ld_ja(a, k + 2 * L);
                const int    c3 = jb + ld_ja(a, k + 3 * L);
                const double v0 = ld_val(a, k);
                const double v1 = ld_val(a, k + L);
                const double v2 = ld_val(a, k + 2 * L);
                const double v3 = ld_val(a, k + 3 * L);
                const double x0 = a.x[c0], x1 = a.x[c1], x2 = a.x[c2], x3 = a.x[c3];
                if (OP == OP_JACOBI) {
                    if (c0 != r) s += v0 * x0;
                    if (c1 != r) s += v1 * x1;
                    if (c2 != r) s += v2 * x2;
                    if (c3 != r) s += v3 * x3;
                } else {
                    s += v0 * x0;
                    s += v1 * x1;
                    s += v2 * x2;
                    s += v3 * x3;
                }
            }
            if (k < ke) {
                const int    kl = ke - 1;
                const int    k1 = min(k + L, kl), k2 = min(k + 2 * L, kl);
                const int    c0 = jb + ld_ja(a, k), c1 = jb + ld_ja(a, k1), c2 = jb + ld_ja(a, k2);
                const double v0 = ld_val(a, k);
                const double w1 = ld_val(a, k1), w2 = ld_val(a, k2);
                const double v1 = (k + L < ke) ? w1 : 0.0, v2 = (k + 2 * L < ke) ? w2 : 0.0;
                const double x0 = a.x[c0], x1 = a.x[c1], x2 = a.x[c2];
                if (OP == OP_JACOBI) {
                    if (c0 != r) s += v0 * x0;
                    if (c1 != r) s += v1 * x1;
                    if (c2 != r) s += v2 * x2;
                } else {
                    s += v0 * x0;
                    s += v1 * x1;
                    s += v2 * x2;
                }
            }
            s = subwave_sum<L>(s);
            if (sl == 0) {
                if (OP == OP_MXV) { a.y[r] = s; zx_store(a, r, s); }
                else if (OP == OP_RESID) a.y[r] = a.b[r] - s;
                else if (OP == OP_ADD) a.y[r] += s;
                else if (OP == OP_SUB) a.y[r] -= s;
// ... 915 lines not shown
```

### faspsolver_amd/csrc/solver.hip

```cpp
#include <hip/hip_runtime.h>

#include <fcntl.h>
#include <omp.h>
#include <sys/mman.h>
#include <sys/stat.h>
#include <unistd.h>

#include <algorithm>
#include <cfloat>
#include <cmath>
#include <cstdio>
#include <cstdlib>
#include <cstring>
#include <functional>
#include <condition_variable>
#include <memory>
#include <mutex>
#include <string>
#include <thread>
#include <type_traits>
#include <vector>

#include "fasp_comm.h"
#include "fasp_internal.h"
#include "krylov_ws.h"
#include "kernels.hip.h"
#include "kernels2.hip.h"
#include "kernels3.hip.h"
#include "kernels4.hip.h"
#include "small_solvers.hip.h"
#include "seq_split.hip.h"
#include "seq_chain.hip.h"

namespace fasp_str { struct CsrSwzDev; }

namespace fasp {

#define HIPCK(expr)                                                                        \
    do {                                                                                   \
        hipError_t e_ = (expr);                                                            \
        if (e_ != hipSuccess) {                                                            \
            std::fprintf(stderr, "### ERROR: fasp_hip: %s failed: %s [%s:%d]\n", #expr,    \
                         hipGetErrorString(e_), __FILE__, __LINE__);                       \
            return ERROR_MISC;                                                             \
        }                                                                                  \
    } while (0)

struct Ctx {
    bool        ready  = false;
    int         device = -1;
    hipStream_t stream = nullptr;
    hipStream_t comm_stream = nullptr;
    hipEvent_t  ev_ready = nullptr, ev_halo = nullptr;
    double*     d_partials = nullptr;
    double*     d_partials2 = nullptr;
    double*     h_part     = nullptr;
    double*     d_red      = nullptr;
    double*     h_red      = nullptr;
    int         num_cu     = 256;
};
static Ctx g_ctx;
static int g_requested_device = -1;

constexpr int RED_SLOTS = 16;

static int ctx_init()
{
    if (g_ctx.ready) return FASP_SUCCESS;
    int ndev = 0;
    hipError_t e = hipGetDeviceCount(&ndev);
    if (e != hipSuccess || ndev <= 0) {
        std::fprintf(stderr, "### ERROR: fasp_hip: no HIP device available (%s). This library has "
                             "no CPU fallback.\n", e == hipSuccess ? "device count 0" : hipGetErrorString(e));
        return ERROR_MISC;
    }
    int dev = 0;
    if (g_requested_device >= 0) dev = g_requested_device;
    else if (const char* lr = std::getenv("FASP_HIP_DEVICE")) dev = std::atoi(lr);
    if (dev < 0 || dev >= ndev) {
        const char* wrap = std::getenv("FASP_HIP_ALLOW_DEVICE_WRAP");
        if (wrap && std::atoi(wrap) != 0 && dev >= 0) dev = dev % ndev;
        else {
            std::fprintf(stderr, "### ERROR: fasp_hip: device %d requested, %d visible (one process per GPU; "
                                 "FASP_HIP_ALLOW_DEVICE_WRAP=1 shares devices for the shared-memory validation transport)\n", dev, ndev);
            return ERROR_INPUT_PAR;
        }
    }
    HIPCK(hipSetDevice(dev));
    hipDeviceProp_t prop;
    HIPCK(hipGetDeviceProperties(&prop, dev));
    if (std::strncmp(prop.gcnArchName, "gfx950", 6) != 0)
        std::fprintf(stderr, "### WARNING: fasp_hip: device %d is %s; kernels are built for gfx950\n",
                     dev, prop.gcnArchName);
    g_ctx.num_cu = prop.multiProcessorCount;
    g_ctx.device = dev;
    HIPCK(hipStreamCreateWithFlags(&g_ctx.stream, hipStreamNonBlocking));
    HIPCK(hipStreamCreateWithFlags(&g_ctx.comm_stream, hipStreamNonBlocking));
    HIPCK(hipEventCreateWithFlags(&g_ctx.ev_ready, hipEventDisableTiming));
    HIPCK(hipEventCreateWithFlags(&g_ctx.ev_halo, hipEventDisableTiming));
    HIPCK(hipMalloc(&g_ctx.d_partials, sizeof(double) * 8 * MAXGRID));
    HIPCK(hipMalloc(&g_ctx.d_partials2, sizeof(double) * (8 * MAXGRID + 8)));
    HIPCK(hipHostMalloc(&g_ctx.h_part, sizeof(double) * (8 * MAXGRID + 8), hipHostMallocDefault));
    HIPCK(hipMalloc(&g_ctx.d_red, sizeof(double) * RED_SLOTS));
    HIPCK(hipHostMalloc(&g_ctx.h_red, sizeof(double) * RED_SLOTS, hipHostMallocDefault));
    g_ctx.ready = true;
    if (const char* tv = std::getenv("FASP_HIP_TUNE")) {
        std::string all(tv);
        size_t p0 = 0;
        while (p0 < all.size()) {
            size_t p1 = all.find(',', p0);
            if (p1 == std::string::npos) p1 = all.size();
            const std::string kv = all.substr(p0, p1 - p0);
            const size_t eq = kv.find('=');
            if (eq != std::string::npos && fasp_hip_tune(kv.substr(0, eq).c_str(), std::atoi(kv.c_str() + eq + 1)) < 0)
                std::fprintf(stderr, "### WARNING: fasp_hip: FASP_HIP_TUNE: unknown key in '%s'\n", kv.c_str());
            p0 = p1 + 1;
        }
    }
    return FASP_SUCCESS;
}

static inline int vec_grid(int n)
{
    long long g = ((long long)n + BLOCK - 1) / BLOCK;
    if (g > MAXGRID) g = MAXGRID;
    if (g < 1) g = 1;
    return (int)g;
}

#include "device_csr.hip.h"

#include "hierarchy.hip.h"

#include "smoothers.hip.h"

#include "coarse_cg.hip.h"

#include "krylov.hip.h"

#include "cycles.hip.h"

#include "pcg.hip.h"

}

#include "bsr.hip.h"
#include "str_common.hip.h"
#include "csr_swz.hip.h"
#include "str.hip.h"
#include "str_ilu.hip.h"
#include "str_sweep.hip.h"
#include "str_swz.hip.h"

static std::recursive_mutex g_entry_mutex;
#define FASP_ENTRY() std::lock_guard<std::recursive_mutex> fasp_entry_lock_(g_entry_mutex)

extern "C" {

int fasp_hip_set_device(int device)
{
    FASP_ENTRY();
    if (g_ctx.ready && device != g_ctx.device) {
        std::fprintf(stderr, "### ERROR: fasp_hip: device already bound to %d\n", g_ctx.device);
        return ERROR_INPUT_PAR;
    }
    g_requested_device = device;
    return ctx_init();
}

int fasp_hip_device_count(void)
{
    FASP_ENTRY();
    int n = 0;
    if (hipGetDeviceCount(&n) != hipSuccess) return ERROR_MISC;
    return n;
}

int fasp_hip_device_identity(char* out, int cap)
{
    FASP_ENTRY();
    if (!out || cap < 16) return ERROR_INPUT_PAR;
    if (ctx_init() < 0) return ERROR_MISC;
// ... 1792 lines not shown
    if (!M.ok) die_bsr(__func__);
    const size_t n = (size_t)A->ROW * A->nb;
    TmpVec du(u->val, n), dun(nullptr, n), db(b->val, n), dd(diaginv, (size_t)A->ROW * A->nb * A->nb);
    BsrArgs a{}; a.x = du.d; a.y = dun.d; a.b = db.d; a.dinv = dd.d;
    launch_bsr<2>(M, a);
    dun.get(u->val);
}

int fasp_hip_bsr_sweep(const dBSRmat* A, const double* b, double* u, const double* diaginv, int descend, int sor, double w,
                       int* nlevels)
{
    FASP_ENTRY();
    if (!A || !b || !u || !diaginv || !nlevels || !A->IA || (A->NNZ > 0 && (!A->JA || !A->val))) return ERROR_INPUT_PAR;
    if (A->nb < 1 || A->nb > 7 || A->storage_manner != 0 || A->ROW != A->COL || A->ROW < 0 || A->NNZ < 0) return ERROR_INPUT_PAR;
    TmpBSR M(A);
    if (!M.ok) return ERROR_MISC;
    const size_t n = (size_t)A->ROW * A->nb;
    TmpVec du(u, n), db(b, n), dd(diaginv, n * A->nb);
    if (!du.d || !db.d || !dd.d) return ERROR_MISC;
    DevLevel::Sched S;
    int st = bsr_seq_schedule(A->ROW, A->COL, A->NNZ, A->IA, A->JA, descend != 0, S);
    if (st >= 0) st = bsr_seq_launch(M, S, db.d, dd.d, du.d, sor != 0, w);
    if (st >= 0) { *nlevels = (int)S.ptr.size() - 1; du.get(u); }
    else (void)hipStreamSynchronize(g_ctx.stream);
    S.release();
    return st;
}

double fasp_hip_time_bsr_mxv(const dBSRmat* A, int reps)
{
    FASP_ENTRY();
    TmpBSR M(A);
    if (!M.ok || reps <= 0) return -1.0;
    TmpVec dx(nullptr, (size_t)A->COL * A->nb), dy(nullptr, (size_t)A->ROW * A->nb);
    (void)hipMemsetAsync(dx.d, 0, sizeof(double) * dx.n, g_ctx.stream);
    BsrArgs a{}; a.x = dx.d; a.y = dy.d;
    hipEvent_t e0, e1;
    (void)hipEventCreate(&e0); (void)hipEventCreate(&e1);
    launch_bsr<0>(M, a); launch_bsr<0>(M, a);
    (void)hipEventRecord(e0, g_ctx.stream);
    for (int i = 0; i < reps; ++i) launch_bsr<0>(M, a);
    (void)hipEventRecord(e1, g_ctx.stream);
    (void)hipEventSynchronize(e1);
    float ms = 0.f;
    (void)hipEventElapsedTime(&ms, e0, e1);
    (void)hipEventDestroy(e0); (void)hipEventDestroy(e1);
    return (double)ms / reps;
}

void fasp_smoother_dcsr_jacobi(dvector* u, const int i_1, const int i_n, const int s, dCSRmat* A, dvector* b,
                               int L, const double w)
{
    FASP_ENTRY();
    (void)s;
    TmpCSR M(A);
    if (!M.ok) die_no_device(__func__);
    const int n = A->row;
    const int lo = std::min(i_1, i_n), hi = std::max(i_1, i_n);
    if (lo != 0 || hi != n - 1) {
        std::fprintf(stderr, "### ERROR: fasp_smoother_dcsr_jacobi (device): only full sweeps 0..n-1 supported\n");
        std::exit(ERROR_INPUT_PAR);
    }
    std::vector<double> d(n, 0.0);
    bool dup = false;
    for (int i = 0; i < n; ++i) {
        int hits = 0;
        for (int k = A->IA[i]; k < A->IA[i + 1]; ++k)
            if (A->JA[k] == i) { d[i] = A->val[k]; ++hits; }
        dup = dup || hits > 1;
    }
    M.D.dup_diag = dup;
    TmpVec du(u->val, n), du2(nullptr, n), db(b->val, n), dd(d.data(), n);
    double *x = du.d, *xo = du2.d;
    while (L--) {
        CsrArgs a{};
        a.x = x; a.y = xo; a.b = db.d; a.diag = dd.d; a.omega = w;
        launch_csr<OP_JACOBI>(M.D, a);
        std::swap(x, xo);
    }
    (void)hipStreamSynchronize(g_ctx.stream);
    (void)hipMemcpy(u->val, x, sizeof(double) * n, hipMemcpyDeviceToHost);
}

#ifdef FLOW_TIMING
extern "C" int fasp_hip_flow_times(unsigned long long* out, int n)
{
    FASP_ENTRY();
    return hipMemcpyFromSymbol(out, HIP_SYMBOL(fasp::g_flow_times), sizeof(unsigned long long) * (size_t)std::min(n, 8192)) == hipSuccess ? 0 : -1;
}
#endif

static int g_time_cold = 0;
int fasp_hip_tune(const char* key, int value)
{
    FASP_ENTRY();
    if (!key) return ERROR_INPUT_PAR;
    if (!std::strcmp(key, "maxgrid")) g_tune.maxgrid = value;
    else if (!std::strcmp(key, "xcd")) g_tune.xcd = value;
    else if (!std::strcmp(key, "gen2")) g_tune.gen2 = value;
    else if (!std::strcmp(key, "ws2_bpc")) g_tune.ws2_bpc = value;
    else if (!std::strcmp(key, "nt")) g_tune.nt = value;
    else if (!std::strcmp(key, "kind")) g_tune.kind = value;
    else if (!std::strcmp(key, "compress")) g_tune.compress = value;
    else if (!std::strcmp(key, "rpl")) g_tune.rpl = value;
    else if (!std::strcmp(key, "lds_tab")) g_tune.lds_tab = value;
    else if (!std::strcmp(key, "xcd_pat")) g_tune.xcd_pat = value;
    else if (!std::strcmp(key, "spcg_batch")) g_tune.spcg_batch = value;
    else if (!std::strcmp(key, "spcg_fused")) g_tune.spcg_fused = value;
    else if (!std::strcmp(key, "spcg_persist")) { g_tune.spcg_persist = value; if (value) g_persist_disabled = false; }
    else if (!std::strcmp(key, "spcg_test_hang")) g_tune.spcg_test_hang = value;
    else if (!std::strcmp(key, "spcg_grid")) g_tune.spcg_grid = value;
    else if (!std::strcmp(key, "small_lds")) g_tune.small_lds = value;
    else if (!std::strcmp(key, "small_onewave")) g_tune.small_onewave = value;
    else if (!std::strcmp(key, "ja16")) g_tune.ja16 = value;
    else if (!std::strcmp(key, "device_sort")) g_device_sort = value;
    else if (!std::strcmp(key, "halo_overlap")) g_halo_overlap = value;
    else if (!std::strcmp(key, "coarse_mode")) g_coarse_mode = value;
    else if (!std::strcmp(key, "coarse_split_min")) g_coarse_split_min = value;
    else if (!std::strcmp(key, "split_rows")) g_tune.split_rows = value;
    else if (!std::strcmp(key, "gs_multicolor")) g_tune.gs_multicolor = value;
    else if (!std::strcmp(key, "seq_flow")) { g_tune.seq_flow = value; if (value) g_flow_disabled = false; }
    else if (!std::strcmp(key, "ilu_smooth_fused")) g_tune.ilu_smooth_fused = value;
    else if (!std::strcmp(key, "swz_run")) g_tune.swz_run = value;
    else if (!std::strcmp(key, "swz_run_width")) g_tune.swz_run_width = value;
    else if (!std::strcmp(key, "ilu_form")) g_tune.ilu_form = value;
    else if (!std::strcmp(key, "str_ilu_form")) g_tune.str_ilu_form = value;
    else if (!std::strcmp(key, "str_ilu_wgs")) g_tune.str_ilu_wgs = value;
    else if (!std::strcmp(key, "str_sweep_form")) g_tune.str_sweep_form = value;
    else if (!std::strcmp(key, "str_sweep_wgs")) g_tune.str_sweep_wgs = value;
    else if (!std::strcmp(key, "seq_strip_kb")) g_tune.seq_strip_kb = value;
    else if (!std::strcmp(key, "seq_jobs")) g_tune.seq_jobs = value;
    else if (!std::strcmp(key, "local_square")) g_tune.local_square = value;
    else if (!std::strcmp(key, "seq_grid")) g_tune.seq_grid = value;
    else if (!std::strcmp(key, "seq_chain")) g_tune.seq_chain = value;
    else if (!std::strcmp(key, "seq_chain_n1")) g_tune.seq_chain_n1 = value;
    else if (!std::strcmp(key, "seq_chain_grid")) g_tune.seq_chain_grid = value;
    else if (!std::strcmp(key, "seq_test_hang")) g_tune.seq_test_hang = value;
    else if (!std::strcmp(key, "seq_rest_lanes")) g_tune.seq_rest_lanes = value;
    else if (!std::strcmp(key, "seq_chain_ref")) g_tune.seq_chain_ref = value;
    else if (!std::strcmp(key, "seq_spine")) g_tune.seq_spine = value;
    else if (!std::strcmp(key, "seq_partition")) g_seq_partition = value;
    else if (!std::strcmp(key, "fuse_zr")) g_tune.fuse_zr = value;
    else if (!std::strcmp(key, "fuse_presmooth")) g_tune.fuse_presmooth = value;
    else if (!std::strcmp(key, "seq_lanes")) g_tune.seq_lanes = value;
    else if (!std::strcmp(key, "lazy_coarse")) g_tune.lazy_coarse = value;
    else if (!std::strcmp(key, "xtile")) g_tune.xtile = value;
    else if (!std::strcmp(key, "rp5_max")) g_tune.rp5_max = value;
    else if (!std::strcmp(key, "rp_bpc")) g_tune.rp_bpc = value;
    else if (!std::strcmp(key, "rp_stream")) g_tune.rp_stream = value;
    else if (!std::strcmp(key, "renumber")) g_tune.renumber = value;
    else if (!std::strcmp(key, "renumber_chunk")) g_tune.renumber_chunk = value;
    else if (!std::strcmp(key, "time_cold")) g_time_cold = value;
    else if (!std::strcmp(key, "estream")) g_tune.estream = value;
    else if (!std::strcmp(key, "sell")) g_tune.sell = value;
    else if (!std::strcmp(key, "es_dbg")) g_tune.es_dbg = value;
    else if (!std::strcmp(key, "pcg_dev_beta")) g_tune.pcg_dev_beta = value;
    else if (!std::strcmp(key, "seq_chain_touch")) g_tune.seq_chain_touch = value;
    else if (!std::strcmp(key, "seq_chain_touch_t1")) g_tune.seq_chain_touch_t1 = value;
    else if (!std::strcmp(key, "seq_zero_skip")) g_tune.seq_zero_skip = value;
    else if (!std::strcmp(key, "pcg_fold")) g_tune.pcg_fold = value;
    else if (!std::strcmp(key, "spcg_spec")) g_tune.spcg_spec = value;
    else if (!std::strcmp(key, "ev_every")) g_tune.ev_every = value;
    else if (!std::strcmp(key, "rp_xcd")) g_tune.rp_xcd = value;
    else if (!std::strcmp(key, "rp_strip")) g_tune.rp_strip = value;
    else if (!std::strcmp(key, "host_parallel_min")) g_parallel_min_nnz = value;
    else if (!std::strcmp(key, "rap_form")) g_rap_form = value;
    else if (!std::strcmp(key, "rap_arena_kb")) g_rap_arena_kb = value;
    else if (!std::strcmp(key, "device_rap")) g_device_rap = value;
    else if (!std::strcmp(key, "lanes")) g_tune.lanes = value;
    else if (!std::strcmp(key, "wrows")) g_tune.wrows = value;
    else if (!std::strcmp(key, "wcap")) g_tune.wcap = value;
    else return ERROR_INPUT_PAR;
    return FASP_SUCCESS;
}

int fasp_hip_sell_selftest(const dCSRmat* A, int cap_percent, int* info, double* bytes, int* ia_out, int* ja_out, double* val_out, const double* x, double* y)
{
    if (!A || !info || A->row < 0 || A->nnz < 0) return ERROR_INPUT_PAR;
    HostCSR M;
    M.row = A->row; M.col = A->col; M.nnz = A->nnz;
    M.ia.view(A->IA, (size_t)A->row + 1); M.ja.view(A->JA, (size_t)std::max(A->nnz, 1)); M.val.view(A->val, (size_t)std::max(A->nnz, 1));
    SellHost S;
    int why = 0;
    const bool ok = build_sell(M, S, cap_percent > 0 ? cap_percent : SELL_CAP_PERCENT, &why);
    info[0] = ok ? 1 : 0; info[1] = why; info[2] = S.nv; info[3] = S.vbits; info[4] = S.obits; info[5] = S.nslice;
    info[6] = ok ? (int)std::min<long long>(S.slots / 64, 0x7fffffff) : 0; info[7] = SELL_MAXV;
    if (bytes) *bytes = ok ? S.bytes(M.row) : 0.0;
    if (!ok) return FASP_SUCCESS;
    if (ia_out && ja_out && val_out) sell_decode_host(S, M.row, ia_out, ja_out, val_out);
    if (x && y) sell_mxv_host(S, M.row, x, y);
    return FASP_SUCCESS;
}

int fasp_hip_csr_plan(const int* traits, int op, int windowed, int want_partials, int* plan, double* bytes)
{
    FASP_ENTRY();
    if (!traits || !plan || op < OP_MXV || op > OP_MXV_DOT) return ERROR_INPUT_PAR;
    static double dummy[1];
    const int* t = traits;
    auto flag = [&](int i) -> void* { return t[i] ? dummy : nullptr; };
    DevCSR M;
    M.row = t[0]; M.col = t[1]; M.nnz = t[2]; M.kind = t[3]; M.lanes = t[4]; M.wrows = t[5]; M.wcap = t[6]; M.nxrows = t[7]; M.plane = t[8];
    M.npat = t[9]; M.npent = t[10]; M.sell_nv = t[11]; M.sell_nslice = t[12]; M.sell_slots = t[13]; M.ntcols = t[14]; M.es_W = t[15]; M.es_nc = t[16];
    M.code = (unsigned char*)flag(17); M.pat = (unsigned short*)flag(18); M.rowbase = (int*)flag(19); M.dpos = (int*)flag(20); M.dup_diag = t[21] != 0;
    M.ja16 = (unsigned short*)flag(22); M.jbase = (int*)flag(23); M.lja16 = (unsigned short*)flag(24); M.sell_code = (unsigned*)flag(25);
    M.es_tab = (int*)flag(26); M.es_ja16 = (unsigned short*)flag(27);
    const CsrPlan p = plan_csr(M, op, windowed || g_tune.split_rows > 0, want_partials != 0);
    const int out[11] = {(int)p.kernel, p.family, p.tile_rows, p.bpc, p.xcd_map, p.tpp, p.nt, p.ja16, p.jbase, p.fused_zr, kernel_family(M, nullptr)};
    std::copy(out, out + 11, plan);
    if (bytes) *bytes = p.bytes;
    return FASP_SUCCESS;
}

int fasp_hip_estream_selftest(const int* ia, int nrow, int nnz, int per_wave, int wmax, int* info)
{
    if (!ia || nrow < 1 || nnz < 1 || per_wave < 8 || wmax < 32) return ERROR_INPUT_PAR;
    return estream_selftest_host(ia, nrow, nnz, per_wave, wmax, info);
}

int fasp_hip_measure_ceilings(double* out, size_t bytes, int reps)
{
    FASP_ENTRY();
    if (!out || bytes < (1u << 20) || reps <= 0) return ERROR_INPUT_PAR;
    if (ctx_init() != FASP_SUCCESS) return ERROR_MISC;
    f64x2_t *p = nullptr, *q = nullptr, *r = nullptr;
    HIPCK(hipMalloc(&p, bytes)); HIPCK(hipMalloc(&q, bytes)); HIPCK(hipMalloc(&r, bytes));
    HIPCK(hipMemsetAsync(p, 0, bytes, g_ctx.stream)); HIPCK(hipMemsetAsync(q, 0, bytes, g_ctx.stream));
    HIPCK(hipMemsetAsync(r, 0, bytes, g_ctx.stream));
    const size_t n16 = bytes / 16;
    hipEvent_t e0, e1;
    HIPCK(hipEventCreate(&e0)); HIPCK(hipEventCreate(&e1));
    const int grid = 4 * g_ctx.num_cu;
    for (int which = 0; which < 3; ++which) {
        auto run = [&]() {
            if (which == 0) hipLaunchKernelGGL(k_read16, dim3(grid), dim3(BLOCK), 0, g_ctx.stream, n16, p, (double*)q);
            else if (which == 1) hipLaunchKernelGGL(k_copy16, dim3(grid), dim3(BLOCK), 0, g_ctx.stream, n16, p, q);
            else hipLaunchKernelGGL(k_triad16, dim3(grid), dim3(BLOCK), 0, g_ctx.stream, n16, 0.5, p, q, r);
        };
        run(); run();
        HIPCK(hipEventRecord(e0, g_ctx.stream));
        for (int i = 0; i < reps; ++i) run();
        HIPCK(hipEventRecord(e1, g_ctx.stream));
        HIPCK(hipEventSynchronize(e1));
        float ms = 0.f;
        HIPCK(hipEventElapsedTime(&ms, e0, e1));
        out[which] = (double)(which + 1) * (double)bytes * reps / ((double)ms * 1e-3) / 1e9;
    }
    (void)hipEventDestroy(e0); (void)hipEventDestroy(e1);
    (void)hipFree(p); (void)hipFree(q); (void)hipFree(r);
    return FASP_SUCCESS;
}

double fasp_hip_time_kernel(fasp_hip_amg* h, int kind, int level, int reps)
{
    FASP_ENTRY();
    if (!h || level < 0 || level >= (int)h->L.size() || reps <= 0) return -1.0;
    DevLevel& D = h->L[level];
    const int n = D.A.row;
    hipEvent_t e0, e1;
    if (hipEventCreate(&e0) != hipSuccess || hipEventCreate(&e1) != hipSuccess) return -1.0;
    double* x = D.xa; double* y = D.xb; double* w = D.w;
    auto run = [&]() {
        switch (kind) {
            case 0: d_mxv(D.A, x, y); break;
            case 1: d_aAxpy(-1.0, D.A, x, y); break;
            case 2: { CsrArgs a{}; a.x = x; a.y = y; a.b = w; a.diag = D.diag; a.omega = 0.6667; launch_csr<OP_JACOBI>(D.A, a); } break;
            case 3: hipLaunchKernelGGL(k_dot, dim3(vec_grid(n)), dim3(BLOCK), 0, g_ctx.stream, n, x, y, g_ctx.d_partials); break;
            case 4: d_axpy(n, 0.5, x, y); break;
            case 5: { CsrArgs a{}; a.x = x; a.y = y; a.dotv = x; a.partials = g_ctx.d_partials; launch_csr<OP_MXV_DOT>(D.A, a); } break;
            case 6: if (D.R.ia) d_mxv(D.R, w, h->L[level + 1].xa); break;
            case 7: if (D.P.ia) d_aAxpy(1.0, D.P, h->L[level + 1].xa, y); break;
            case 8:
                if (D.A.val) hipLaunchKernelGGL(k_read16, dim3(2048), dim3(BLOCK), 0, g_ctx.stream, (size_t)D.A.nnz / 2, (const f64x2_t*)D.A.val, y);
                break;
            case 10: case 11: case 12: case 13: (void)seq_sweep(h, level, kind - 10, 1, 1.0); break;
            default: break;
        }
    };
    (void)hipMemsetAsync(x, 0, sizeof(double) * n, g_ctx.stream);
    (void)hipMemsetAsync(y, 0, sizeof(double) * n, g_ctx.stream);
    (void)hipMemsetAsync(w, 0, sizeof(double) * n, g_ctx.stream);
    double* const keep_b = D.b; double* const keep_x = D.x;
    if (kind >= 10) { D.b = w; D.x = x; }
    if (g_time_cold) {
        double* big = nullptr;
        const size_t bigb = (size_t)512 << 20;
        if (hipMalloc(&big, bigb + 4096) != hipSuccess) return -1.0;
        (void)hipMemsetAsync(big, 0, bigb, g_ctx.stream);
        double tot = 0.0;
        for (int i = 0; i < reps + 1; ++i) {
            if (g_time_cold >= 2) (void)hipMemsetAsync(big, 0, bigb, g_ctx.stream);
            else hipLaunchKernelGGL(k_read16, dim3(1024), dim3(BLOCK), 0, g_ctx.stream, bigb / 16, (const f64x2_t*)big, big + bigb / 8);
            (void)hipEventRecord(e0, g_ctx.stream);
            run();
            (void)hipEventRecord(e1, g_ctx.stream);
            (void)hipEventSynchronize(e1);
            float ms1 = 0.f;
            (void)hipEventElapsedTime(&ms1, e0, e1);
            if (i >= 1) tot += ms1;
        }
        (void)hipFree(big);
        D.b = keep_b; D.x = keep_x;
        (void)hipEventDestroy(e0); (void)hipEventDestroy(e1);
        return tot / reps;
    }
    run(); run();
    (void)hipEventRecord(e0, g_ctx.stream);
    for (int i = 0; i < reps; ++i) run();
    (void)hipEventRecord(e1, g_ctx.stream);
    (void)hipEventSynchronize(e1);
    D.b = keep_b; D.x = keep_x;
    float ms = 0.f;
    (void)hipEventElapsedTime(&ms, e0, e1);
    (void)hipEventDestroy(e0); (void)hipEventDestroy(e1);
    return (double)ms / reps;
}


static int row_op_host(DevLevel& D, int which, int op, const double* x, const double* b, double* y, double* y2, double scalar, double* red)
{
    if (which < 0 || which > 2 || op < 0 || op > 8 || !x || !y) return ERROR_INPUT_PAR;
    const DevCSR& M = which == 0 ? D.A : which == 1 ? D.P : D.R;
    if (!M.ia || ((op == 5 || op == 6) && which != 0) || ((op == 1 || op >= 5) && !b) || (op == 8 && !y2)) return ERROR_INPUT_PAR;
    const size_t nr = (size_t)std::max(M.row, 1), nc = (size_t)std::max(M.col, 1);
    double *dx = nullptr, *db = nullptr, *dy = nullptr, *dy2 = nullptr;
    int st = FASP_SUCCESS;
    auto run = [&]() -> int {
        HIPCK(hipMalloc(&dx, 8 * nc)); HIPCK(hipMalloc(&db, 8 * nr)); HIPCK(hipMalloc(&dy, 8 * nr)); HIPCK(hipMalloc(&dy2, 8 * nr));
        HIPCK(hipMemcpy(dx, x, 8 * (size_t)M.col, hipMemcpyHostToDevice));
        HIPCK(hipMemcpy(dy, y, 8 * (size_t)M.row, hipMemcpyHostToDevice));
        if (b) HIPCK(hipMemcpy(db, b, 8 * (size_t)M.row, hipMemcpyHostToDevice));
        CsrArgs a{};
        a.x = dx; a.y = dy; a.b = db;
        int G = 0;
        bool have_red = false;
        switch (op) {
            case 0: G = launch_csr<OP_MXV>(M, a); break;
            case 1: G = launch_csr<OP_RESID>(M, a); break;
            case 2: G = launch_csr<OP_ADD>(M, a); break;
            case 3: G = launch_csr<OP_SUB>(M, a); break;
            case 4: a.alpha = scalar; G = launch_csr<OP_AXPY>(M, a); break;
            case 5:
                a.diag = D.diag; a.omega = scalar;
                if (red) a.partials = g_ctx.d_partials;
                G = launch_csr<OP_JACOBI>(M, a);
                have_red = red && plan_csr(M, OP_JACOBI, false, true).fused_zr;
                break;
            case 6: a.diag = D.l1; a.omega = scalar; G = launch_csr<OP_L1DIAG>(M, a); break;
            case 7: a.b = nullptr; a.dotv = db; a.partials = g_ctx.d_partials; G = launch_csr<OP_MXV_DOT>(M, a); have_red = red != nullptr; break;
            default: a.b = nullptr; a.zx = dy2; a.zdiag = db; a.zomega = scalar; G = launch_csr<OP_MXV>(M, a); break;
        }
        if (red) *red = std::nan("");
        if (have_red) {
            d_finalize(G, 1, 0u, 0, false);
            if (fetch_red(0, 1, red) < 0) return ERROR_MISC;
        }
        HIPCK(hipStreamSynchronize(g_ctx.stream));
        HIPCK(hipMemcpy(y, dy, 8 * (size_t)M.row, hipMemcpyDeviceToHost));
        if (op == 8) HIPCK(hipMemcpy(y2, dy2, 8 * (size_t)M.row, hipMemcpyDeviceToHost));
        return FASP_SUCCESS;
    };
    st = run();
    (void)hipFree(dx); (void)hipFree(db); (void)hipFree(dy); (void)hipFree(dy2);
    return st;
}

int fasp_hip_level_op(fasp_hip_amg* h, int level, int which, int op, const double* x, const double* b, double* y, double* y2, double scalar, double* red)
{
    FASP_ENTRY();
    if (!h || level < 0 || level >= (int)h->L.size()) return ERROR_INPUT_PAR;
    return row_op_host(h->L[level], which, op, x, b, y, y2, scalar, red);
}
int fasp_hip_matrix_op(const dCSRmat* A, int op, const double* x, const double* b, double* y, double* y2, double scalar, double* red, int* kind_out)
{
    FASP_ENTRY();
    if (!A || ctx_init() < 0) return ERROR_INPUT_PAR;
    HostCSR M;
    M.row = A->row; M.col = A->col; M.nnz = A->nnz;
    M.ia.view(A->IA, (size_t)A->row + 1); M.ja.view(A->JA, (size_t)std::max(A->nnz, 1)); M.val.view(A->val, (size_t)std::max(A->nnz, 1));
    DevLevel D;
    int st;
    {
        HostThreads team;
        st = upload_csr(M, D.A);
        if (st >= 0 && M.row == M.col) st = upload_diag(M, D);
    }
    if (st >= 0 && (op == 5 || op == 6) && !D.diag) st = ERROR_INPUT_PAR;
    if (st >= 0) st = row_op_host(D, 0, op, x, b, y, y2, scalar, red);
    if (kind_out) *kind_out = kernel_family(D.A, nullptr);
    free_level(D);
    return st;
}

int fasp_hip_matrix_traits(const dCSRmat* A, int* traits)
{
    FASP_ENTRY();
    if (!A || !traits || ctx_init() < 0) return ERROR_INPUT_PAR;
    HostCSR M;
    M.row = A->row; M.col = A->col; M.nnz = A->nnz;
    M.ia.view(A->IA, (size_t)A->row + 1); M.ja.view(A->JA, (size_t)std::max(A->nnz, 1)); M.val.view(A->val, (size_t)std::max(A->nnz, 1));
    DevLevel D;
    int st;
    {
        HostThreads team;
        st = upload_csr(M, D.A);
        if (st >= 0 && M.row == M.col) st = upload_diag(M, D);
    }
    if (st >= 0) {
        const DevCSR& d = D.A;
        const int out[28] = {d.row, d.col, d.nnz, d.kind, d.lanes, d.wrows, d.wcap, d.nxrows, d.plane, d.npat, d.npent, d.sell_nv, d.sell_nslice,
                             (int)d.sell_slots, (int)d.ntcols, d.es_W, d.es_nc, d.code != nullptr, d.pat != nullptr, d.rowbase != nullptr, d.dpos != nullptr,
                             d.dup_diag, d.ja16 != nullptr, d.jbase != nullptr, d.lja16 != nullptr, d.sell_code != nullptr, d.es_tab != nullptr, d.es_ja16 != nullptr};
        std::copy(out, out + 28, traits);
    }
    free_level(D);
    return st < 0 ? st : FASP_SUCCESS;
}

double fasp_hip_time_matrix(const dCSRmat* A, int op, int reps, int* kind_out)
{
    FASP_ENTRY();
    if (!A || reps <= 0 || ctx_init() < 0) return -1.0;
    HostCSR M;
    M.row = A->row; M.col = A->col; M.nnz = A->nnz;
    M.row_aligned = A->col > A->row && std::getenv("FASP_HIP_TIME_ROW_ALIGNED") != nullptr;
    M.ia.view(A->IA, (size_t)A->row + 1); M.ja.view(A->JA, (size_t)std::max(A->nnz, 1)); M.val.view(A->val, (size_t)std::max(A->nnz, 1));
    DevCSR D;
    {
        HostThreads team;
        if (upload_csr(M, D) < 0) { D.release(); return -1.0; }
    }
    const int n = A->row, nc = A->col;
    double *x = nullptr, *y = nullptr, *w = nullptr, *dg = nullptr;
    if (hipMalloc(&x, 8 * (size_t)std::max(nc, n)) != hipSuccess || hipMalloc(&y, 8 * (size_t)n) != hipSuccess ||
        hipMalloc(&w, 8 * (size_t)n) != hipSuccess || hipMalloc(&dg, 8 * (size_t)n) != hipSuccess) { D.release(); return -1.0; }
    (void)hipMemsetAsync(x, 0, 8 * (size_t)std::max(nc, n), g_ctx.stream);
    (void)hipMemsetAsync(y, 0, 8 * (size_t)n, g_ctx.stream);
    (void)hipMemsetAsync(w, 0, 8 * (size_t)n, g_ctx.stream);
    hipLaunchKernelGGL(k_set, dim3(vec_grid(n)), dim3(BLOCK), 0, g_ctx.stream, n, 1.0, dg);
    const int row_op = op == 0 ? OP_MXV : op == 1 ? OP_SUB : op == 2 ? OP_JACOBI : OP_MXV_DOT;
    auto run = [&]() {
        switch (row_op) {
            case OP_MXV: d_mxv(D, x, y); break;
            case OP_SUB: d_aAxpy(-1.0, D, x, y); break;
            case OP_JACOBI: { CsrArgs a{}; a.x = x; a.y = y; a.b = w; a.diag = dg; a.omega = 0.6667; launch_csr<OP_JACOBI>(D, a); } break;
            default: { CsrArgs a{}; a.x = x; a.y = y; a.dotv = x; a.partials = g_ctx.d_partials; launch_csr<OP_MXV_DOT>(D, a); } break;
        }
    };
    hipEvent_t e0, e1;
    (void)hipEventCreate(&e0); (void)hipEventCreate(&e1);
    run(); run();
    (void)hipEventRecord(e0, g_ctx.stream);
    for (int i = 0; i < reps; ++i) run();
    (void)hipEventRecord(e1, g_ctx.stream);
    (void)hipEventSynchronize(e1);
    float ms = 0.f;
    (void)hipEventElapsedTime(&ms, e0, e1);
    (void)hipEventDestroy(e0); (void)hipEventDestroy(e1);
    if (kind_out) *kind_out = plan_csr(D, row_op, g_tune.split_rows > 0, false).family;
    (void)hipFree(x); (void)hipFree(y); (void)hipFree(w); (void)hipFree(dg);
    D.release();
    return (double)ms / reps;
}

}
```

### include/fasp_hip_dev.h

```cpp
#ifndef FASP_HIP_DEV_H
#define FASP_HIP_DEV_H
#include "fasp_hip.h"
#ifdef __cplusplus
extern "C" {
#endif

double fasp_hip_time_kernel(fasp_hip_amg* h, int kind, int level, int reps);
double fasp_hip_time_matrix(const dCSRmat* A, int op, int reps, int* kind_out);
double fasp_hip_seq_schedule_selftest(const dCSRmat* A, const int* seq, int ns, int strip_kb, int lanes, int spine, int* info);
int fasp_hip_cluster_order(const dCSRmat* A, int chunk, int* order);
int fasp_hip_permute_csr(const dCSRmat* A, const int* rperm, const int* cinv, int* ia, int* ja, double* val);
double fasp_hip_seq_chain_selftest(const dCSRmat* A, const int* seq, int ns, int n1_blocks, int form, double w, int* info, double* out_u);
int fasp_hip_measure_ceilings(double* out, size_t bytes, int reps);

int    fasp_hip_ilu_resident_count(void);
double fasp_hip_ilu_time(ILU_data* iludata, int which, int reps, double* info);
int    fasp_hip_bsr_amg_get_ilu(const fasp_hip_amg_bsr* h, int level, ILU_data* view);
int    fasp_hip_bsr_amg_ilu_info(const fasp_hip_amg_bsr* h, int level, double info[6]);
double fasp_hip_bsr_amg_ilu_smooth_time(fasp_hip_amg_bsr* h, int level, int reps);

int    fasp_hip_dcsr_rap(const dCSRmat* R, const dCSRmat* A, const dCSRmat* P, dCSRmat* RAP);
int    fasp_hip_rap_info(int info[4]);
long   fasp_hip_rap_device_count(void);
double fasp_hip_rap_time(const dCSRmat* R, const dCSRmat* A, const dCSRmat* P, int where, int reps);

int fasp_hip_tune(const char* key, int value);
int fasp_hip_coarse_kernel_info(const fasp_hip_amg* h, int* info);
int fasp_hip_bsr_coarse_kernel_info(const fasp_hip_amg_bsr* h, int* info);

int fasp_hip_comm_stats(double* out8, int reset);
int fasp_hip_comm_timing(int on);

int fasp_hip_dist_plan(fasp_hip_amg* h, int rank, int nranks, int min_rows);
int fasp_hip_dist_level_info(const fasp_hip_amg* h, int level, int* info);
int fasp_hip_dist_get_matrix(const fasp_hip_amg* h, int level, int which, dCSRmat* view);
int fasp_hip_dist_get_list(const fasp_hip_amg* h, int level, int which, ivector* view);
int  fasp_hip_estream_selftest(const int* ia, int nrow, int nnz, int per_wave, int wmax, int* info);
int  fasp_hip_csr_plan(const int* traits, int op, int windowed, int want_partials, int* plan, double* bytes);
int  fasp_hip_sell_selftest(const dCSRmat* A, int cap_percent, int* info, double* bytes, int* ia_out, int* ja_out, double* val_out, const double* x, double* y);
int  fasp_hip_level_op(fasp_hip_amg* h, int level, int which, int op, const double* x, const double* b, double* y, double* y2, double scalar, double* red);
int  fasp_hip_matrix_op(const dCSRmat* A, int op, const double* x, const double* b, double* y, double* y2, double scalar, double* red, int* kind_out);
int  fasp_hip_matrix_traits(const dCSRmat* A, int* traits);
int  fasp_hip_bsr_sweep(const dBSRmat* A, const double* b, double* u, const double* diaginv, int descend, int sor, double w, int* nlevels);
int  fasp_hip_csr_sweep(const dCSRmat* A, const int* seq, int ns, int form, double w, int zero_start, const double* b, double* u, int* info);
int  fasp_hip_str_form(const dSTRmat* A);
double fasp_hip_time_str_mxv(const dSTRmat* A, int reps);
int    fasp_hip_str_ilu_form(const dSTRmat* LU, int lfil);
int    fasp_hip_str_ilu_apply(const dSTRmat* LU, int lfil, const double* r, double* z);
double fasp_hip_time_str_ilu(const dSTRmat* LU, int lfil, int reps);
int    fasp_hip_str_sweep(const dSTRmat* A, int kind, int order, const int* mark, double weight, const double* diaginv, const double* b,
                          double* u, int nsweeps, int* info);
int    fasp_hip_str_sweep_form(const dSTRmat* A, int order, const int* mark);
int    fasp_hip_str_sweep_levels(const dSTRmat* A, int order, const int* mark, int* visit, int* level, int cap);
double fasp_hip_time_str_sweep(const dSTRmat* A, int kind, int order, const int* mark, double weight, int reps);
int  fasp_hip_str_swz(const dSTRmat* A, const int* neigh, int nneigh, const int* order, const double* b, double* u, int nsweeps, int* info);
int  fasp_hip_str_swz_levels(const dSTRmat* A, const int* neigh, int nneigh, const int* order, int* visit, int* level, int cap);
int  fasp_hip_time_str_swz(const dSTRmat* A, const int* neigh, int nneigh, const int* order, int reps, double* ms_factor, double* ms_sweep, int* info);
int  fasp_hip_csr_swz_levels(const SWZ_data* swz, int backward, int* level, int cap);
int  fasp_hip_csr_swz(SWZ_data* swz, int dir, const double* b, double* x, int nsweeps, int* info, double* fac, int* piv);
int  fasp_hip_csr_swz_resident_count(void);
int  fasp_hip_time_csr_swz(SWZ_data* swz, int reps, double* ms, double* bytes, int* info);
int    fasp_hip_csr_swz_runs(const SWZ_data* swz, int backward, int width, int* run_first, int cap);
int    fasp_hip_amg_get_swz(const fasp_hip_amg* h, int level, SWZ_data* view);
int    fasp_hip_amg_swz_levels(const fasp_hip_amg* h, int level, int* swz_levels);
int    fasp_hip_amg_swz_info(const fasp_hip_amg* h, int level, int* info);
double fasp_hip_amg_swz_sweep_time(fasp_hip_amg* h, int level, int dir, int reps);
int  fasp_hip_comm_selftest(void);

#ifdef __cplusplus
}
#endif
#endif
```

Before: 475.8 million.

## Add row-group compressed CSR format and kernels for dense-row matrices

Adds a new sparse format that packs groups of 8 or 16 rows sharing column indices into 16-bit offsets plus row-membership bitmasks, with new multi-wave SpMV kernels and planner selection. The aim is to cut index bandwidth for matrices averaging at least 128 nonzeros per row through column reuse across rows. For the 7-point Poisson fine grid (about 7 nnz per row) it is gated off, so only dense coarse AMG levels could use it. This adds extra setup time and device memory for the coded copy.

```diff
diff --git a/faspsolver_amd/__init__.py b/faspsolver_amd/__init__.py
--- a/faspsolver_amd/__init__.py
+++ b/faspsolver_amd/__init__.py
@@ -39,7 +39,7 @@
     "fasp_hip_dist_get_list",
     "fasp_blas_dcsr_vmv", "fasp_blas_dcsr_mxv_agg", "fasp_blas_dcsr_aAxpy_agg", "fasp_blas_darray_ax",
     "fasp_blas_darray_axpyz", "fasp_blas_darray_norm1", "fasp_darray_cp", "fasp_darray_set", "fasp_dvec_isnan",
-    "fasp_hip_time_matrix", "fasp_hip_bsr_dist_info", "fasp_hip_seq_schedule_selftest", "fasp_hip_seq_chain_selftest", "fasp_hip_cluster_order", "fasp_hip_permute_csr", "fasp_hip_comm_init_ipc", "fasp_hip_comm_stats", "fasp_hip_comm_timing", "fasp_hip_estream_selftest", "fasp_hip_sell_selftest", "fasp_hip_csr_plan", "fasp_hip_level_op", "fasp_hip_matrix_op", "fasp_hip_matrix_traits",
+    "fasp_hip_time_matrix", "fasp_hip_bsr_dist_info", "fasp_hip_seq_schedule_selftest", "fasp_hip_seq_chain_selftest", "fasp_hip_cluster_order", "fasp_hip_permute_csr", "fasp_hip_comm_init_ipc", "fasp_hip_comm_stats", "fasp_hip_comm_timing", "fasp_hip_estream_selftest", "fasp_hip_sell_selftest", "fasp_hip_csr_plan", "fasp_hip_level_op", "fasp_hip_matrix_op", "fasp_hip_matrix_traits", "fasp_hip_matrix_traits2", "fasp_hip_csr_plan2", "fasp_hip_rgroup_selftest",
     "fasp_param_ilu_init", "fasp_ilu_data_create", "fasp_ilu_data_free", "fasp_mem_iludata_check", "fasp_ilu_dcsr_setup",
     "fasp_precond_ilu", "fasp_precond_ilu_forward", "fasp_precond_ilu_backward", "fasp_solver_dcsr_krylov_ilu",
     "fasp_solver_dcsr_krylov_ilu_M", "fasp_smoother_dcsr_ilu", "fasp_fwrapper_dcsr_krylov_ilu_",
diff --git a/faspsolver_amd/csrc/device_csr.hip.h b/faspsolver_amd/csrc/device_csr.hip.h
--- a/faspsolver_amd/csrc/device_csr.hip.h
+++ b/faspsolver_amd/csrc/device_csr.hip.h
@@ -43,8 +43,17 @@
     double*        sell_tab = nullptr;
     int            sell_nv = 0, sell_obits = 0, sell_nslice = 0;
     long long      sell_slots = 0;
+    unsigned*      rg_code = nullptr;
+    double*        rg_val = nullptr;
+    int*           rg_meta = nullptr;
+    int            rg_R = 0, rg_ng = 0;
+    long long      rg_words = 0;
     void    release()
     {
+        if (rg_code) (void)hipFree(rg_code);
+        if (rg_val) (void)hipFree(rg_val);
+        if (rg_meta) (void)hipFree(rg_meta);
+        rg_code = nullptr; rg_val = nullptr; rg_meta = nullptr; rg_R = rg_ng = 0; rg_words = 0;
         if (sell_code) (void)hipFree(sell_code);
         if (sell_meta) (void)hipFree(sell_meta);
         if (sell_rlen) (void)hipFree(sell_rlen);
@@ -829,6 +838,177 @@
             const unsigned c = cs[(size_t)k * 64 + l];
             ja[ia[r] + k] = base + (int)(c & omask);
             val[ia[r] + k] = S.tab[c >> S.obits];
+        }
+    }
+}
+
+constexpr int    RG_MIN_ROW   = 128;
+constexpr int    RG_ROWS      = 8;
+constexpr double RG_W4_MIN_ROW = 256.0, RG_W8_MIN_ROW = 1000.0;
+constexpr double RG_MIN_REUSE = 3.0;
+struct RGroupHost {
+    int R = 0, ng = 0;
+    long long words = 0, chunks = 0, ucols = 0;
+    std::vector<int> meta;
+    Buf<unsigned>    code;
+    Buf<double>      val;
+};
+static double rgroup_bytes(long long nnz, long long words, int ng) { return 8.0 * (double)nnz + 4.0 * (double)words + 16.0 * (ng + 1.0); }
+static bool build_rgroup(const HostCSR& M, int R, double min_reuse, RGroupHost& G, int* why_not)
+{
+    int dummy = 0;
+    int& why = why_not ? *why_not : dummy;
+    G = RGroupHost();
+    G.R = R;
+    if (M.row != M.col) { why = 1; return false; }
+    if (M.row <= 0 || M.nnz <= 0 || (double)M.nnz < (double)RG_MIN_ROW * M.row) { why = 2; return false; }
+    const int n = M.row, ng = (n + R - 1) / R, sh = 32 - R;
+    std::vector<std::vector<unsigned>> gcode((size_t)ng);
+    std::vector<int> gbase((size_t)ng, 0), gnch((size_t)ng, 0);
+    G.val.alloc((size_t)M.nnz + 2);
+    G.val[(size_t)M.nnz] = 0.0; G.val[(size_t)M.nnz + 1] = 0.0;
+    int bad = 0;
+#pragma omp parallel
+    {
+        std::vector<unsigned> mask((size_t)65536, 0u);
+        std::vector<int>      pos((size_t)65536, 0);
+        std::vector<unsigned short> touched;
+        std::vector<int> slot;
+        int mybad = 0;
+#pragma omp for schedule(dynamic, 16)
+        for (int g = 0; g < ng; ++g) {
+            const int r0 = g * R, r1 = std::min(n, r0 + R), k0 = M.ia[r0], k1 = M.ia[r1];
+            std::vector<unsigned>& out = gcode[(size_t)g];
+            if (k1 <= k0) { out.assign(1, 0u); continue; }
+            int lo = M.ja[k0], hi = lo;
+            for (int k = k0 + 1; k < k1; ++k) { lo = std::min(lo, M.ja[k]); hi = std::max(hi, M.ja[k]); }
+            if (hi - lo > 65535) { mybad = mybad ? std::min(mybad, 3) : 3; continue; }
+            gbase[(size_t)g] = lo;
+            touched.clear();
+            bool dup = false;
+            for (int r = r0; r < r1; ++r)
+                for (int k = M.ia[r]; k < M.ia[r + 1]; ++k) {
+                    const int off = M.ja[k] - lo;
+                    const unsigned bit = 1u << (r - r0);
+                    if (!mask[(size_t)off]) touched.push_back((unsigned short)off);
+                    if (mask[(size_t)off] & bit) dup = true;
+                    mask[(size_t)off] |= bit;
+                }
+            if (dup) {
+                mybad = mybad ? std::min(mybad, 4) : 4;
+                for (unsigned short t : touched) mask[t] = 0u;
+                continue;
+            }
+            std::sort(touched.begin(), touched.end());
+            const int nu = (int)touched.size(), nch = (nu + 63) / 64;
+            out.resize((size_t)nch + 1 + nu);
+            gnch[(size_t)g] = nch;
+            slot.assign((size_t)nu * R, -1);
+            int next = 0;
+            for (int c = 0; c < nch; ++c) {
+                out[(size_t)c] = (unsigned)next;
+                const int u1 = std::min(nu, 64 * c + 64);
+                for (int r = 0; r < R; ++r)
+                    for (int u = 64 * c; u < u1; ++u)
+                        if (mask[touched[(size_t)u]] >> r & 1u) slot[(size_t)u * R + r] = next++;
+            }
+            out[(size_t)nch] = (unsigned)next;
+            for (int u = 0; u < nu; ++u) {
+                pos[touched[(size_t)u]] = u;
+                out[(size_t)nch + 1 + u] = (unsigned)touched[(size_t)u] | (mask[touched[(size_t)u]] << sh);
+            }
+            for (int r = r0; r < r1; ++r)
+                for (int k = M.ia[r]; k < M.ia[r + 1]; ++k)
+                    G.val[(size_t)k0 + (size_t)slot[(size_t)pos[(size_t)(M.ja[k] - lo)] * R + (r - r0)]] = M.val[k];
+            for (unsigned short t : touched) mask[t] = 0u;
+        }
+#pragma omp critical
+        if (mybad) bad = bad ? std::min(bad, mybad) : mybad;
+    }
+    if (bad) { why = bad; return false; }
+    G.ng = ng;
+    G.meta.assign(4 * ((size_t)ng + 1), 0);
+    long long w = 0;
+    for (int g = 0; g < ng; ++g) {
+        const std::vector<unsigned>& c = gcode[(size_t)g];
+        const int r0 = g * R;
+        const int nch = gnch[(size_t)g];
+        G.meta[4 * (size_t)g] = (int)w; G.meta[4 * (size_t)g + 1] = M.ia[r0]; G.meta[4 * (size_t)g + 2] = gbase[(size_t)g]; G.meta[4 * (size_t)g + 3] = nch;
+        w += (long long)c.size();
+        G.chunks += nch;
+        G.ucols += (long long)c.size() - (nch + 1);
+    }
+    if (w >= (1ll << 31) - 8) { why = 2; return false; }
+    G.meta[4 * (size_t)ng] = (int)w; G.meta[4 * (size_t)ng + 1] = M.nnz;
+    G.words = w;
+    if ((double)M.nnz < min_reuse * (double)G.ucols) { why = 5; return false; }
+    G.code.alloc((size_t)((w + 3) & ~3ll) + 4);
+    for (long long i = w; i < ((w + 3) & ~3ll) + 4; ++i) G.code[(size_t)i] = 0u;
+#pragma omp parallel for schedule(static)
+    for (int g = 0; g < ng; ++g) std::copy(gcode[(size_t)g].begin(), gcode[(size_t)g].end(), G.code.data() + G.meta[4 * (size_t)g]);
+    why = 0;
+    return true;
+}
+static void rgroup_mxv_host(const RGroupHost& G, int nrow, int NW, const double* x, double* y)
+{
+    const int R = G.R, sh = 32 - R;
+    for (int g = 0; g < G.ng; ++g) {
+        const int woff = G.meta[4 * (size_t)g], voff = G.meta[4 * (size_t)g + 1], cbase = G.meta[4 * (size_t)g + 2], nch = G.meta[4 * (size_t)g + 3];
+        const int len = G.meta[4 * (size_t)g + 4] - woff - (nch + 1);
+        const unsigned* coff = G.code.data() + woff;
+        const unsigned* wd = coff + nch + 1;
+        double sum[16][64];
+        for (int w = 0; w < NW; ++w) {
+            double acc[16][64];
+            for (int r = 0; r < R; ++r)
+                for (int l = 0; l < 64; ++l) acc[r][l] = 0.0;
+            for (int c = nch * w / NW; c < nch * (w + 1) / NW; ++c) {
+                int at = voff + (int)coff[c];
+                for (int r = 0; r < R; ++r)
+                    for (int l = 0; l < 64 && 64 * c + l < len; ++l) {
+                        const unsigned word = wd[64 * c + l];
+                        if (!((word >> (sh + r)) & 1u)) continue;
+                        const double p = G.val[(size_t)at++] * x[cbase + (int)(word & 0xffffu)];
+                        acc[r][l] = acc[r][l] + p;
+                    }
+            }
+            for (int r = 0; r < R; ++r)
+                for (int l = 0; l < 64; ++l) sum[r][l] = w == 0 ? acc[r][l] : sum[r][l] + acc[r][l];
+        }
+        for (int r = 0; r < R && g * R + r < nrow; ++r) {
+            double* v = sum[r];
+            double t[64];
+            for (int s = 1; s <= 8; s <<= 1) {
+                for (int l = 0; l < 64; ++l) t[l] = v[l] + ((l & 15) >= s ? v[l - s] : 0.0);
+                for (int l = 0; l < 64; ++l) v[l] = t[l];
+            }
+            for (int l = 0; l < 64; ++l) t[l] = v[l] + (((l >> 4) & 1) ? v[(l & ~15) - 1] : 0.0);
+            for (int l = 0; l < 64; ++l) v[l] = t[l];
+            for (int l = 0; l < 64; ++l) t[l] = v[l] + (l >= 32 ? v[31] : 0.0);
+            y[g * R + r] = t[63];
+        }
+    }
+}
+static void rgroup_decode_host(const RGroupHost& G, int nrow, int* ia, int* ja, double* val)
+{
+    const int R = G.R, sh = 32 - R;
+    int k = 0;
+    ia[0] = 0;
+    for (int g = 0; g < G.ng; ++g) {
+        const int woff = G.meta[4 * (size_t)g], voff = G.meta[4 * (size_t)g + 1], cbase = G.meta[4 * (size_t)g + 2], nch = G.meta[4 * (size_t)g + 3];
+        const int len = G.meta[4 * (size_t)g + 4] - woff - (nch + 1);
+        const unsigned* coff = G.code.data() + woff;
+        const unsigned* wd = coff + nch + 1;
+        for (int r = 0; r < R && g * R + r < nrow; ++r) {
+            for (int c = 0; c < nch; ++c) {
+                int at = voff + (int)coff[c];
+                const int u1 = std::min(len, 64 * c + 64);
+                for (int q = 0; q < r; ++q)
+                    for (int u = 64 * c; u < u1; ++u) at += (int)((wd[u] >> (sh + q)) & 1u);
+                for (int u = 64 * c; u < u1; ++u)
+                    if ((wd[u] >> (sh + r)) & 1u) { ja[k] = cbase + (int)(wd[u] & 0xffffu); val[k] = G.val[(size_t)at++]; ++k; }
+            }
+            ia[g * R + r + 1] = k;
         }
     }
 }
@@ -1005,8 +1185,32 @@
     return build_estream(H.ia.data(), H.row, H.nnz, D);
 }
 
-struct Tuning { int swz_run = -1, swz_run_width = 16, ilu_smooth_fused = 1, gen2 = 2, ws2_bpc = 3, maxgrid = -1, xcd = 16, nt = 1, kind = -1, lanes = -1, wrows = -1, wcap = -1, compress = 1, rpl = -1, lds_tab = 1, xcd_pat = 64, spcg_batch = 16, small_lds = 1, ja16 = 1, spcg_fused = 1, spcg_grid = 0, spcg_persist = 1, split_rows = 0, gs_multicolor = 0, seq_flow = 1, seq_strip_kb = 0, seq_jobs = 1, seq_spine = 1, seq_grid = 0, seq_chain = 1, seq_chain_n1 = 0, seq_chain_grid = 0, seq_chain_ref = 0, seq_test_hang = 0, seq_rest_lanes = 0, local_square = 1, fuse_zr = 1, fuse_presmooth = 1, seq_lanes = 0, xtile = 1, rp5_max = 45, rp_bpc = 5, rp_xcd = -1, rp_strip = 2, spcg_test_hang = 0, small_onewave = 4, lazy_coarse = 1, rp_stream = -1, renumber = 1, renumber_chunk = 262144, pcg_dev_beta = 1, spcg_spec = 1, ev_every = 4, pcg_fold = 1, seq_chain_touch = 8, seq_chain_touch_t1 = 1, seq_zero_skip = 1, estream = 1, es_dbg = 0, ilu_form = -1, str_ilu_form = -1, str_ilu_wgs = 0, str_sweep_form = -1, str_sweep_wgs = 0, sell = 1; };
+struct Tuning { int swz_run = -1, swz_run_width = 16, ilu_smooth_fused = 1, gen2 = 2, ws2_bpc = 3, maxgrid = -1, xcd = 16, nt = 1, kind = -1, lanes = -1, wrows = -1, wcap = -1, compress = 1, rpl = -1, lds_tab = 1, xcd_pat = 64, spcg_batch = 16, small_lds = 1, ja16 = 1, spcg_fused = 1, spcg_grid = 0, spcg_persist = 1, split_rows = 0, gs_multicolor = 0, seq_flow = 1, seq_strip_kb = 0, seq_jobs = 1, seq_spine = 1, seq_grid = 0, seq_chain = 1, seq_chain_n1 = 0, seq_chain_grid = 0, seq_chain_ref = 0, seq_test_hang = 0, seq_rest_lanes = 0, local_square = 1, fuse_zr = 1, fuse_presmooth = 1, seq_lanes = 0, xtile = 1, rp5_max = 45, rp_bpc = 5, rp_xcd = -1, rp_strip = 2, spcg_test_hang = 0, small_onewave = 4, lazy_coarse = 1, rp_stream = -1, renumber = 1, renumber_chunk = 262144, pcg_dev_beta = 1, spcg_spec = 1, ev_every = 4, pcg_fold = 1, seq_chain_touch = 8, seq_chain_touch_t1 = 1, seq_zero_skip = 1, estream = 1, es_dbg = 0, ilu_form = -1, str_ilu_form = -1, str_ilu_wgs = 0, str_sweep_form = -1, str_sweep_wgs = 0, sell = 1, rgroup = 1, rgroup_rows = 0, rgroup_waves = 0; };
 static Tuning g_tune;
+
+static int upload_rgroup(const HostCSR& H, DevCSR& D)
+{
+    if (g_tune.rgroup == 0 || g_oneshot_upload || H.row != H.col || (double)H.nnz < (double)RG_MIN_ROW * H.row) return FASP_SUCCESS;
+    static const bool timing = std::getenv("FASP_HIP_SETUP_TIMING") != nullptr;
+    const double t0 = wall_seconds();
+    RGroupHost G;
+    int why = 0;
+    const bool ok = build_rgroup(H, g_tune.rgroup_rows == 16 ? 16 : RG_ROWS, RG_MIN_REUSE, G, &why);
+    if (timing) std::printf("        [row groups %d x %d, %d nnz] %s (%d) R %d, %d groups, %lld chunks, reuse %.2f, %.2f bytes per entry, %.3f s\n", H.row, H.col, H.nnz,
+                            ok ? "coded" : "not coded", why, G.R, G.ng, G.chunks, G.ucols ? (double)H.nnz / (double)G.ucols : 0.0,
+                            ok ? rgroup_bytes(H.nnz, G.words, G.ng) / H.nnz : 0.0, wall_seconds() - t0);
+    if (!ok) return FASP_SUCCESS;
+    const size_t nw = (size_t)((G.words + 3) & ~3ll) + 4;
+    HIPCK(hipMalloc(&D.rg_code, sizeof(unsigned) * nw));
+    HIPCK(hipMalloc(&D.rg_val, sizeof(double) * ((size_t)H.nnz + 2)));
+    HIPCK(hipMalloc(&D.rg_meta, sizeof(int) * G.meta.size()));
+    HIPCK(hipMemcpy(D.rg_code, G.code.data(), sizeof(unsigned) * nw, hipMemcpyHostToDevice));
+    HIPCK(hipMemcpy(D.rg_val, G.val.data(), sizeof(double) * ((size_t)H.nnz + 2), hipMemcpyHostToDevice));
+    HIPCK(hipMemcpy(D.rg_meta, G.meta.data(), sizeof(int) * G.meta.size(), hipMemcpyHostToDevice));
+    D.rg_R = G.R; D.rg_ng = G.ng; D.rg_words = G.words;
+    if (timing) std::printf("        [row groups %d x %d] with the copy to the device %.3f s\n", H.row, H.col, wall_seconds() - t0);
+    return FASP_SUCCESS;
+}
 
 template <class K>
 static int resident_blocks_per_cu(K kernel)
@@ -1034,13 +1238,26 @@
     return grid;
 }
 
+static int rgroup_waves_auto(const DevCSR& M)
+{
+    const double avg = M.row > 0 ? (double)M.nnz / M.row : 0.0;
+    return avg >= RG_W8_MIN_ROW ? 8 : avg >= RG_W4_MIN_ROW ? 4 : 2;
+}
+static bool rgroup_measured_faster(const DevCSR& M)
+{
+    const double avg = M.row > 0 ? (double)M.nnz / M.row : 0.0;
+    return M.rg_R == 8 || (avg >= 256.0 && avg < 1200.0);
+}
+
 enum CsrKernel : int {
     CK_ROWS_2 = 0, CK_ROWS_4, CK_ROWS_8, CK_ROWS_16, CK_ROWS_32, CK_ROWS_64,
     CK_WSTREAM_64_512, CK_WSTREAM_64_1024, CK_WSTREAM_32_512, CK_WSTREAM_32_1024,
     CK_ROWPAT_0_1, CK_ROWPAT_0_2, CK_ROWPAT_1_1, CK_ROWPAT_1_2, CK_ROWPAT_2_1, CK_ROWPAT_2_2,
     CK_DICT8_8, CK_DICT8_16, CK_DICT8_24,
     CK_ESTREAM_4, CK_ESTREAM_8, CK_ESTREAM_16, CK_ESTREAM_32,
-    CK_ROWPAT4, CK_ROWPAT5, CK_LSTREAM, CK_XTILE, CK_SELL, CK_WSTREAM2
+    CK_ROWPAT4, CK_ROWPAT5, CK_LSTREAM, CK_XTILE, CK_SELL, CK_WSTREAM2,
+    CK_RGROUP_16_4, CK_RGROUP_16_8, CK_RGROUP_8_4, CK_RGROUP_8_8,
+    CK_RGROUP_16_2, CK_RGROUP_8_2
 };
 struct CsrPlan {
     CsrKernel kernel;
@@ -1121,7 +1338,15 @@
     else {
         if (p.ja16) p.bytes = 10.0 * M.nnz + ptr_bytes + (p.jbase ? 4.0 * M.row : 0.0);
         const bool es_rule = g_tune.estream >= 2 || (g_tune.estream == 1 && (double)M.nnz < 256.0 * M.row);
-        if (M.es_tab && es_rule && p.ja16 && !windowed && op != OP_MXV_DOT && !(jac && (want_partials || M.dup_diag)))
+        const bool rg_rule = g_tune.rgroup >= 2 || (g_tune.rgroup == 1 && g_tune.estream != 0 && rgroup_measured_faster(M));
+        if (M.rg_code && rg_rule && !windowed && op != OP_MXV_DOT && !(jac && (want_partials || M.dup_diag))) {
+            const int tw = g_tune.rgroup_waves, nw = tw == 2 || tw == 4 || tw == 8 ? tw : rgroup_waves_auto(M);
+            p.kernel = M.rg_R == 8 ? (nw == 2 ? CK_RGROUP_8_2 : nw == 4 ? CK_RGROUP_8_4 : CK_RGROUP_8_8) : (nw == 2 ? CK_RGROUP_16_2 : nw == 4 ? CK_RGROUP_16_4 : CK_RGROUP_16_8);
+            p.tile_rows = M.rg_R;
+            p.ja16 = p.jbase = false;
+            p.bytes = rgroup_bytes(M.nnz, M.rg_words, M.rg_ng);
+        }
+        else if (M.es_tab && es_rule && p.ja16 && !windowed && op != OP_MXV_DOT && !(jac && (want_partials || M.dup_diag)))
             p.kernel = avg >= 512.0 ? CK_ESTREAM_32 : avg >= 256.0 ? CK_ESTREAM_16 : avg >= 128.0 ? CK_ESTREAM_8 : CK_ESTREAM_4;
         else
             p.kernel = lanes == 2 ? CK_ROWS_2 : lanes == 4 ? CK_ROWS_4 : lanes == 8 ? CK_ROWS_8 : lanes == 16 ? CK_ROWS_16 : lanes == 32 ? CK_ROWS_32 : CK_ROWS_64;
@@ -1162,6 +1387,24 @@
     grid = std::max(8, (grid + 7) / 8 * 8);
     hipLaunchKernelGGL(k_csr_sell<OP>, dim3(grid), dim3(SELL_BLOCK), lds, g_ctx.stream, a);
     return grid;
+}
+
+template <int R, int NW, int OP>
+static int launch_rgroup(const DevCSR& M, CsrArgs& a)
+{
+    if constexpr (OP == OP_MXV_DOT) { (void)M; (void)a; return 0; }
+    else {
+        a.rg_code = M.rg_code; a.rg_val = M.rg_val; a.rg_meta = M.rg_meta; a.rg_ng = M.rg_ng;
+        constexpr int lds = NW * 64 * R * 8;
+        static bool attr_set = false;
+        if (!attr_set) {
+            (void)hipFuncSetAttribute(reinterpret_cast<const void*>(k_csr_rgroup<R, NW, OP>), hipFuncAttributeMaxDynamicSharedMemorySize, lds);
+            attr_set = true;
+        }
+        const int grid = 8 * ((M.rg_ng + 7) / 8);
+        hipLaunchKernelGGL((k_csr_rgroup<R, NW, OP>), dim3(grid), dim3(NW * 64), lds, g_ctx.stream, a);
+        return grid;
+    }
 }
 
 template <int OP>
@@ -1270,6 +1513,12 @@
         case CK_XTILE:    PERSIST(k_csr_xtile<OP>);
         case CK_SELL:     return launch_sell<OP>(M, a);
         case CK_WSTREAM2: PERSIST(k_csr_wstream2<OP>);
+        case CK_RGROUP_16_4: return launch_rgroup<16, 4, OP>(M, a);
+        case CK_RGROUP_16_8: return launch_rgroup<16, 8, OP>(M, a);
+        case CK_RGROUP_8_4:  return launch_rgroup<8, 4, OP>(M, a);
+        case CK_RGROUP_8_8:  return launch_rgroup<8, 8, OP>(M, a);
+        case CK_RGROUP_16_2: return launch_rgroup<16, 2, OP>(M, a);
+        case CK_RGROUP_8_2:  return launch_rgroup<8, 2, OP>(M, a);
         default: break;
     }
 #undef PERSIST
diff --git a/faspsolver_amd/csrc/hierarchy.hip.h b/faspsolver_amd/csrc/hierarchy.hip.h
--- a/faspsolver_amd/csrc/hierarchy.hip.h
+++ b/faspsolver_amd/csrc/hierarchy.hip.h
@@ -372,6 +372,8 @@
         if (!uploaded && upload_csr(*Adev, D.A) < 0) return ERROR_ALLOC_MEM;
     }
     lap("A");
+    if (rep && HL.has_coarse && upload_rgroup(*Adev, D.A) < 0) return ERROR_ALLOC_MEM;
+    lap("row groups");
     if (renum) {
         if (l > 0 && h->H.L[(size_t)l - 1].has_coarse && !h->L[(size_t)l - 1].P.ia) {
             const int st = upload_transfer(h, l - 1, nullptr);
diff --git a/faspsolver_amd/csrc/kernels.hip.h b/faspsolver_amd/csrc/kernels.hip.h
--- a/faspsolver_amd/csrc/kernels.hip.h
+++ b/faspsolver_amd/csrc/kernels.hip.h
@@ -74,6 +74,10 @@
     const unsigned char* sell_rlen;
     const double*        sell_tab;
     int                  sell_nv, sell_obits;
+    const unsigned*      rg_code;
+    const double*        rg_val;
+    const int*           rg_meta;
+    int                  rg_ng;
 };
 
 __device__ __forceinline__ void zx_store(const CsrArgs& a, int r, double s)
diff --git a/faspsolver_amd/csrc/kernels5.hip.h b/faspsolver_amd/csrc/kernels5.hip.h
--- /dev/null
+++ b/faspsolver_amd/csrc/kernels5.hip.h
@@ -0,0 +1,94 @@
+#pragma once
+
+#include "kernels3.hip.h"
+
+namespace fasp {
+
+template <int R, int NW, int OP>
+__global__ __launch_bounds__(NW * 64) void k_csr_rgroup(CsrArgs a)
+{
+    if (a.stop && *a.stop) return;
+    constexpr int SLAB = 64 * R, NQ = SLAB / 128, SH = 32 - R;
+    static_assert((R == 8 || R == 16) && (NW == 2 || NW == 4 || NW == 8), "rows per group, waves per group");
+    extern __shared__ __attribute__((aligned(16))) double rg_lds[];
+    const int lane = threadIdx.x & 63, wave = __builtin_amdgcn_readfirstlane(threadIdx.x >> 6);
+    const int per = (int)gridDim.x >> 3;
+    const int g = __builtin_amdgcn_readfirstlane((int)(blockIdx.x & 7) * per + (int)(blockIdx.x >> 3));
+    if (g >= a.rg_ng) return;
+    const int woff = es_tab(a.rg_meta, 4 * g), voff = es_tab(a.rg_meta, 4 * g + 1), cbase = es_tab(a.rg_meta, 4 * g + 2), nch = es_tab(a.rg_meta, 4 * g + 3);
+    const int len = es_tab(a.rg_meta, 4 * g + 4) - woff - (nch + 1);
+    const int* const coff = reinterpret_cast<const int*>(a.rg_code) + woff;
+    const __amdgpu_buffer_rsrc_t rw = __builtin_amdgcn_make_buffer_rsrc(const_cast<unsigned*>(a.rg_code) + woff + nch + 1, 0, len * 4, 0x00020000);
+    double* const sv = rg_lds + wave * SLAB;
+    const int c_lo = nch * wave / NW, c_hi = nch * (wave + 1) / NW;
+
+    auto load_word = [&](int c) { return (unsigned)__builtin_amdgcn_raw_buffer_load_b32(rw, (c * 64 + lane) * 4, 0, 0); };
+    f64x2_t qv[NQ];
+    auto stage_load = [&](int vo, int n) {
+        const __amdgpu_buffer_rsrc_t rv = __builtin_amdgcn_make_buffer_rsrc(const_cast<double*>(a.rg_val) + vo, 0, ((n + 1) & ~1) * 8, 0x00020000);
+#pragma unroll
+        for (int q = 0; q < NQ; ++q)
+            if (q * 128 < n) qv[q] = __builtin_bit_cast(f64x2_t, __builtin_amdgcn_raw_buffer_load_b128(rv, (lane + 64 * q) * 16, 0, 0));
+    };
+    auto stage_store = [&](int n) {
+#pragma unroll
+        for (int q = 0; q < NQ; ++q)
+            if (q * 128 < n) reinterpret_cast<f64x2_t*>(sv)[lane + 64 * q] = qv[q];
+    };
+
+    double acc[R];
+#pragma unroll
+    for (int r = 0; r < R; ++r) acc[r] = 0.0;
+    if (c_lo < c_hi) {
+        int v0 = voff + es_tab(coff, c_lo), v1 = voff + es_tab(coff, c_lo + 1);
+        unsigned wcur = load_word(c_lo), wnext = load_word(c_lo + 1);
+        stage_load(v0, v1 - v0);
+        double xcur = a.x[cbase + (int)(wcur & 0xffffu)];
+        stage_store(v1 - v0);
+        wave_order();
+        for (int c = c_lo; c < c_hi; ++c) {
+            const bool more = c + 1 < c_hi;
+            const int  v2 = more ? voff + es_tab(coff, c + 2) : v1;
+            const unsigned wn2   = load_word(c + 2);
+            const double   xnext = a.x[cbase + (int)(wnext & 0xffffu)];
+            stage_load(v1, v2 - v1);
+            int rb = 0;
+            double vv[R];
+#pragma unroll
+            for (int r = 0; r < R; ++r) {
+                const unsigned long long m = __builtin_amdgcn_ballot_w64(((wcur >> (SH + r)) & 1u) != 0u);
+                const int rank = (int)__builtin_amdgcn_mbcnt_hi((unsigned)(m >> 32), __builtin_amdgcn_mbcnt_lo((unsigned)m, 0u));
+                vv[r] = sv[rb + rank];
+                rb += __builtin_popcountll(m);
+            }
+#pragma unroll
+            for (int r = 0; r < R; ++r) {
+                const double p = vv[r] * xcur;
+                acc[r] = acc[r] + (((wcur >> (SH + r)) & 1u) != 0u ? p : 0.0);
+            }
+            wave_order();
+            stage_store(v2 - v1);
+            wave_order();
+            wcur = wnext; wnext = wn2; xcur = xnext; v0 = v1; v1 = v2;
+        }
+    }
+    wave_order();
+#pragma unroll
+    for (int r = 0; r < R; ++r) sv[r * 64 + lane] = acc[r];
+    __syncthreads();
+    constexpr int PP = R / NW > 0 ? R / NW : 1;
+    if (wave * PP < R) {
+#pragma unroll
+        for (int j = 0; j < PP; ++j) {
+            const int r = wave * PP + j;
+            double s = rg_lds[r * 64 + lane];
+#pragma unroll
+            for (int q = 1; q < NW; ++q) s += rg_lds[q * SLAB + r * 64 + lane];
+            s = es_group_sum<64>(s);
+            const int row = g * R + r;
+            if (lane == 63 && row < a.nrow) es_epilogue<OP>(a, row, s);
+        }
+    }
+}
+
+}
diff --git a/faspsolver_amd/csrc/solver.hip b/faspsolver_amd/csrc/solver.hip
--- a/faspsolver_amd/csrc/solver.hip
+++ b/faspsolver_amd/csrc/solver.hip
@@ -28,6 +28,7 @@
 #include "kernels2.hip.h"
 #include "kernels3.hip.h"
 #include "kernels4.hip.h"
+#include "kernels5.hip.h"
 #include "small_solvers.hip.h"
 #include "seq_split.hip.h"
 #include "seq_chain.hip.h"
@@ -2126,6 +2127,9 @@
     else if (!std::strcmp(key, "renumber_chunk")) g_tune.renumber_chunk = value;
     else if (!std::strcmp(key, "time_cold")) g_time_cold = value;
     else if (!std::strcmp(key, "estream")) g_tune.estream = value;
+    else if (!std::strcmp(key, "rgroup")) g_tune.rgroup = value;
+    else if (!std::strcmp(key, "rgroup_rows")) g_tune.rgroup_rows = value;
+    else if (!std::strcmp(key, "rgroup_waves")) g_tune.rgroup_waves = value;
     else if (!std::strcmp(key, "sell")) g_tune.sell = value;
     else if (!std::strcmp(key, "es_dbg")) g_tune.es_dbg = value;
     else if (!std::strcmp(key, "pcg_dev_beta")) g_tune.pcg_dev_beta = value;
@@ -2183,6 +2187,48 @@
     const int out[11] = {(int)p.kernel, p.family, p.tile_rows, p.bpc, p.xcd_map, p.tpp, p.nt, p.ja16, p.jbase, p.fused_zr, kernel_family(M, nullptr)};
     std::copy(out, out + 11, plan);
     if (bytes) *bytes = p.bytes;
+    return FASP_SUCCESS;
+}
+
+int fasp_hip_csr_plan2(const int* traits, int op, int windowed, int want_partials, int* plan, double* bytes)
+{
+    FASP_ENTRY();
+    if (!traits || !plan || op < OP_MXV || op > OP_MXV_DOT) return ERROR_INPUT_PAR;
+    static double dummy[1];
+    const int* t = traits;
+    auto flag = [&](int i) -> void* { return t[i] ? dummy : nullptr; };
+    DevCSR M;
+    M.row = t[0]; M.col = t[1]; M.nnz = t[2]; M.kind = t[3]; M.lanes = t[4]; M.wrows = t[5]; M.wcap = t[6]; M.nxrows = t[7]; M.plane = t[8];
+    M.npat = t[9]; M.npent = t[10]; M.sell_nv = t[11]; M.sell_nslice = t[12]; M.sell_slots = t[13]; M.ntcols = t[14]; M.es_W = t[15]; M.es_nc = t[16];
+    M.code = (unsigned char*)flag(17); M.pat = (unsigned short*)flag(18); M.rowbase = (int*)flag(19); M.dpos = (int*)flag(20); M.dup_diag = t[21] != 0;
+    M.ja16 = (unsigned short*)flag(22); M.jbase = (int*)flag(23); M.lja16 = (unsigned short*)flag(24); M.sell_code = (unsigned*)flag(25);
+    M.es_tab = (int*)flag(26); M.es_ja16 = (unsigned short*)flag(27);
+    M.rg_code = (unsigned*)flag(28); M.rg_R = t[29]; M.rg_ng = t[30]; M.rg_words = t[31];
+    const CsrPlan p = plan_csr(M, op, windowed || g_tune.split_rows > 0, want_partials != 0);
+    const int out[11] = {(int)p.kernel, p.family, p.tile_rows, p.bpc, p.xcd_map, p.tpp, p.nt, p.ja16, p.jbase, p.fused_zr, kernel_family(M, nullptr)};
+    std::copy(out, out + 11, plan);
+    if (bytes) *bytes = p.bytes;
+    return FASP_SUCCESS;
+}
+
+int fasp_hip_rgroup_selftest(const dCSRmat* A, int rows_per_group, int waves, double min_reuse, int* info, double* bytes, int* ia_out, int* ja_out, double* val_out, const double* x, double* y)
+{
+    if (!A || !info || A->row < 0 || A->nnz < 0 || (rows_per_group != 8 && rows_per_group != 16) || (waves != 2 && waves != 4 && waves != 8)) return ERROR_INPUT_PAR;
+    HostCSR M;
+    M.row = A->row; M.col = A->col; M.nnz = A->nnz;
+    M.ia.view(A->IA, (size_t)A->row + 1); M.ja.view(A->JA, (size_t)std::max(A->nnz, 1)); M.val.view(A->val, (size_t)std::max(A->nnz, 1));
+    RGroupHost G;
+    int why = 0;
+    const bool ok = build_rgroup(M, rows_per_group, min_reuse > 0.0 ? min_reuse : RG_MIN_REUSE, G, &why);
+    unsigned long long hsh = 1469598103934665603ull;
+    auto eat = [&](const void* p, size_t n) { const unsigned char* q = (const unsigned char*)p; for (size_t i = 0; i < n; ++i) { hsh ^= q[i]; hsh *= 1099511628211ull; } };
+    if (ok) { eat(G.meta.data(), 4 * G.meta.size()); eat(G.code.data(), 4 * (size_t)(((G.words + 3) & ~3ll) + 4)); eat(G.val.data(), 8 * ((size_t)M.nnz + 2)); }
+    info[0] = ok ? 1 : 0; info[1] = why; info[2] = G.R; info[3] = G.ng; info[4] = (int)G.chunks; info[5] = (int)G.ucols; info[6] = (int)G.words;
+    info[7] = (int)(hsh & 0x7fffffffu); info[8] = (int)((hsh >> 32) & 0x7fffffffu); info[9] = RG_MIN_ROW;
+    if (bytes) *bytes = ok ? rgroup_bytes(M.nnz, G.words, G.ng) : 0.0;
+    if (!ok) return FASP_SUCCESS;
+    if (ia_out && ja_out && val_out) rgroup_decode_host(G, M.row, ia_out, ja_out, val_out);
+    if (x && y) rgroup_mxv_host(G, M.row, waves, x, y);
     return FASP_SUCCESS;
 }
 
@@ -2357,6 +2403,7 @@
     {
         HostThreads team;
         st = upload_csr(M, D.A);
+        if (st >= 0) st = upload_rgroup(M, D.A);
         if (st >= 0 && M.row == M.col) st = upload_diag(M, D);
     }
     if (st >= 0 && (op == 5 || op == 6) && !D.diag) st = ERROR_INPUT_PAR;
@@ -2378,6 +2425,7 @@
     {
         HostThreads team;
         st = upload_csr(M, D.A);
+        if (st >= 0) st = upload_rgroup(M, D.A);
         if (st >= 0 && M.row == M.col) st = upload_diag(M, D);
     }
     if (st >= 0) {
@@ -2386,6 +2434,33 @@
                              (int)d.sell_slots, (int)d.ntcols, d.es_W, d.es_nc, d.code != nullptr, d.pat != nullptr, d.rowbase != nullptr, d.dpos != nullptr,
                              d.dup_diag, d.ja16 != nullptr, d.jbase != nullptr, d.lja16 != nullptr, d.sell_code != nullptr, d.es_tab != nullptr, d.es_ja16 != nullptr};
         std::copy(out, out + 28, traits);
+    }
+    free_level(D);
+    return st < 0 ? st : FASP_SUCCESS;
+}
+
+int fasp_hip_matrix_traits2(const dCSRmat* A, int* traits)
+{
+    FASP_ENTRY();
+    if (!A || !traits || ctx_init() < 0) return ERROR_INPUT_PAR;
+    HostCSR M;
+    M.row = A->row; M.col = A->col; M.nnz = A->nnz;
+    M.ia.view(A->IA, (size_t)A->row + 1); M.ja.view(A->JA, (size_t)std::max(A->nnz, 1)); M.val.view(A->val, (size_t)std::max(A->nnz, 1));
+    DevLevel D;
+    int st;
+    {
+        HostThreads team;
+        st = upload_csr(M, D.A);
+        if (st >= 0) st = upload_rgroup(M, D.A);
+        if (st >= 0 && M.row == M.col) st = upload_diag(M, D);
+    }
+    if (st >= 0) {
+        const DevCSR& d = D.A;
+        const int out[32] = {d.row, d.col, d.nnz, d.kind, d.lanes, d.wrows, d.wcap, d.nxrows, d.plane, d.npat, d.npent, d.sell_nv, d.sell_nslice,
+                             (int)d.sell_slots, (int)d.ntcols, d.es_W, d.es_nc, d.code != nullptr, d.pat != nullptr, d.rowbase != nullptr, d.dpos != nullptr,
+                             d.dup_diag, d.ja16 != nullptr, d.jbase != nullptr, d.lja16 != nullptr, d.sell_code != nullptr, d.es_tab != nullptr, d.es_ja16 != nullptr,
+                             d.rg_code != nullptr, d.rg_R, d.rg_ng, (int)d.rg_words};
+        std::copy(out, out + 32, traits);
     }
     free_level(D);
     return st < 0 ? st : FASP_SUCCESS;
@@ -2402,7 +2477,7 @@
     DevCSR D;
     {
         HostThreads team;
-        if (upload_csr(M, D) < 0) { D.release(); return -1.0; }
+        if (upload_csr(M, D) < 0 || upload_rgroup(M, D) < 0) { D.release(); return -1.0; }
     }
     const int n = A->row, nc = A->col;
     double *x = nullptr, *y = nullptr, *w = nullptr, *dg = nullptr;
diff --git a/include/fasp_hip_dev.h b/include/fasp_hip_dev.h
--- a/include/fasp_hip_dev.h
+++ b/include/fasp_hip_dev.h
@@ -41,6 +41,9 @@
 int  fasp_hip_level_op(fasp_hip_amg* h, int level, int which, int op, const double* x, const double* b, double* y, double* y2, double scalar, double* red);
 int  fasp_hip_matrix_op(const dCSRmat* A, int op, const double* x, const double* b, double* y, double* y2, double scalar, double* red, int* kind_out);
 int  fasp_hip_matrix_traits(const dCSRmat* A, int* traits);
+int  fasp_hip_csr_plan2(const int* traits, int op, int windowed, int want_partials, int* plan, double* bytes);
+int  fasp_hip_matrix_traits2(const dCSRmat* A, int* traits);
+int  fasp_hip_rgroup_selftest(const dCSRmat* A, int rows_per_group, int waves, double min_reuse, int* info, double* bytes, int* ia_out, int* ja_out, double* val_out, const double* x, double* y);
 int  fasp_hip_bsr_sweep(const dBSRmat* A, const double* b, double* u, const double* diaginv, int descend, int sor, double w, int* nlevels);
 int  fasp_hip_csr_sweep(const dCSRmat* A, const int* seq, int ns, int form, double w, int zero_start, const double* b, double* u, int* info);
 int  fasp_hip_str_form(const dSTRmat* A);
```

Measured after the change: 501.7 million, median of 6. 1.05x the previous value.
